# RikVoorhaar/tt-sketch

Hardware: AMD Instinct MI355X
Metric: TT-cores sketched/sec (fp64) + achieved MFMA % for d=6 n=200 r=50 stream_sketch (higher is better)
Workload: dtype f64

## Files before the change

### include/ttsk.h

```cpp
#ifndef TTSK_H
#define TTSK_H

#include <stddef.h>
#include <stdint.h>

#ifdef __cplusplus
extern "C" {
#endif

typedef enum {
    TTSK_OK = 0,
    TTSK_ERR_HIP = -1,
    TTSK_ERR_ARG = -2,
    TTSK_ERR_UNSUPPORTED = -3,
    TTSK_ERR_COMM = -4
} ttsk_status;

#define TTSK_NUM_STREAMS 8

int ttsk_init(int device);
int ttsk_shutdown(void);
const char *ttsk_last_error(void);
int ttsk_device_info(char *name, size_t name_len, int *num_cu, size_t *hbm_bytes);
int ttsk_malloc(void **dev, size_t bytes);
int ttsk_free(void *dev);
int ttsk_memset(void *dev, int value, size_t bytes, int stream);
int ttsk_h2d(void *dev, const void *host, size_t bytes, int stream);
int ttsk_d2h(void *host, const void *dev, size_t bytes, int stream);
int ttsk_d2d(void *dst, const void *src, size_t bytes, int stream);
int ttsk_sync(int stream);
int ttsk_stream_wait(int waiter, int signaller);
int ttsk_timer_start(int stream);
int ttsk_timer_stop(int stream, float *ms);
int ttsk_graph_begin(int stream);
int ttsk_graph_end(int stream, void **graph_exec);
int ttsk_graph_launch(void *graph_exec, int stream);
int ttsk_graph_free(void *graph_exec);

typedef struct {
    int64_t batch, M, N, Ko, Ki;
    int64_t a_b, a_m, a_ko, a_ki;
    int64_t b_b, b_ko, b_ki, b_n;
    int64_t c_b, c_m, c_n;
    double alpha;
    int accumulate;
    int split_k;
} ttsk_gemm_desc;
int ttsk_gemm(const ttsk_gemm_desc *desc, const double *A, const double *B, double *C,
              const double *k_scale ,
              int stream);
int ttsk_copy_strided(double *dst, const double *src, int ndim, const int64_t *shape,
                      const int64_t *dst_strides, const int64_t *src_strides, int stream);
int ttsk_axpby(double *y, const double *x, double a, double b, size_t n, int stream);
int ttsk_sum_slices(double *dst, const double *src, int nb, size_t stride, size_t n, int accumulate, int stream);

int ttsk_tt_sketch(int d, const int64_t *n, const int64_t *s, const int64_t *lt, const int64_t *l_lo,
                   const int64_t *l_hi, const int64_t *rt, const int64_t *r_lo, const int64_t *r_hi,
                   const double *const *X, const double *const *DL, const double *const *DR,
                   double *out, int accumulate, int stream);
int ttsk_tt_sketch_batch(int nb, int d, const int64_t *n, const int64_t *s, const int64_t *lt, const int64_t *l_lo,
                         const int64_t *l_hi, const int64_t *rt, const int64_t *r_lo, const int64_t *r_hi,
                         const double *const *X, const double *const *DL, const double *const *DR,
                         double *out, int64_t out_stride, int accumulate, int stream);
int ttsk_tt_sketch_sum(int nb, int d, const int64_t *n, const int64_t *s, const int64_t *lt, const int64_t *l_lo,
                       const int64_t *l_hi, const int64_t *rt, const int64_t *r_lo, const int64_t *r_hi,
                       const double *const *X, const double *const *DL, const double *const *DR,
                       double *out, int accumulate, int stream);
int ttsk_chain_step(int nb, int n, int K1, int A, int A2, int J, const double *const *W, int64_t w_c,
                    const double *const *X, int64_t x_j, int64_t x_k, int64_t x_c, int64_t x_extent,
                    const double *E, double *const *T, double *const *Out, int stream);
int ttsk_chain_step_wide(int nb, int n, int K1, int A, int A2, int J, const double *const *W, int64_t w_c,
                         const double *const *X, int64_t x_j, int64_t x_k, int64_t x_c, int64_t x_extent,
                         const double *E, double *const *T, double *const *Out, int stream);
int ttsk_chain_step_sum(int nb, int n, int K1, int A, int A2, int J, const double *const *W, int64_t w_c,
                        const double *const *X, int64_t x_j, int64_t x_k, int64_t x_c, int64_t x_extent,
                        const double *E, double *T, int64_t t_b, int64_t t_ld, int64_t t_extent,
                        double *const *Out, int stream);
int ttsk_psi_stream(int nb, int J, int K1, int A, const double *const *S, int64_t s_j, const double *const *W,
                    int64_t w_c, double *const *C, int64_t c_j, int accumulate, int stream);
int ttsk_psi_stream_sum(int nb, int J, int K1, int A, const double *S, int64_t s_j, int64_t s_b, const double *W,
                        int64_t w_c, int64_t w_b, double *C, int64_t c_j, int accumulate, int stream);
int ttsk_drm_pack(const double *core, int A, int n, int A2, int stream);
int ttsk_drm_unpack(const double *core);
int ttsk_dense_left_pass(const double *X, int64_t n0, int64_t n1, int64_t n2, int64_t C, int64_t n4, int l,
                         const double *A0, const double *A1t, const double *A2t, const double *A3, double *Z0, double *Z1,
                         double *Z2, double *E3, int stream);
int64_t ttsk_tt_sketch_size(int d, const int64_t *n, const int64_t *l_lo, const int64_t *l_hi,
                            const int64_t *r_lo, const int64_t *r_hi);
int ttsk_prof_enable(int on);
int ttsk_mfma_f64_peak_probe(double *tflops);
int ttsk_ndtri_rate_probe(double *gsamples);
int ttsk_prof_read(int cls, int64_t *launches, double *total_ms, double *flops);
int ttsk_prof_kernel_name(int cls, char *buf, size_t len);

int ttsk_hash_u64(uint64_t *host_vals, size_t n);
int ttsk_inds_to_rand_double(const uint64_t *host_idx, const uint64_t *shape, int m, size_t N,
                             int rank_min, int rank_max, uint64_t seed, double *host_out);
int ttsk_inds_to_normal(const int64_t *host_idx, const uint64_t *shape, int m, size_t N,
                        int rank_min, int rank_max, uint64_t seed, double *host_out );
int ttsk_inds_to_sparse_sign(const int64_t *host_idx, const uint64_t *shape, int m, size_t N,
                             int true_rank, int rank_min, int rank_max, int nnz_per_row,
                             uint64_t seed, int16_t *host_out );
int ttsk_sparse_normal_dev(const int64_t *dev_idx, int64_t row_stride, const int *row_order,
                           const uint64_t *shape, int m, size_t N, int rank_min, int rank_max,
                           uint64_t seed, double *dev_out, int stream);
int ttsk_sparse_normal_table(const uint64_t *shape, int m, int rank_min, int rank_max, uint64_t seed, double *dev_out,
                             int stream);
int ttsk_sparse_sign_dev(const int64_t *dev_idx, int64_t row_stride, const int *row_order,
                         const uint64_t *shape, int m, size_t N, int true_rank, int rank_min,
                         int rank_max, int nnz_per_row, uint64_t seed, double *dev_out, int stream);
int ttsk_sparse_sign_table(const uint64_t *shape, int m, int true_rank, int rank_min, int rank_max, int nnz_per_row, uint64_t seed,
                           double *dev_out, int stream);
int ttsk_fill_normal(double *dev_out, size_t n, uint64_t seed, double scale, int stream);
int ttsk_fill_normal_many(int count, double *const *dev_outs, const size_t *ns, const uint64_t *seeds,
                          const double *scales, int stream);

int ttsk_sparse_ttdrm_step(const double *dev_vin, int64_t rho, const double *dev_core,
                           int64_t n, int64_t rhop, const int64_t *dev_idx_row, size_t N,
                           double *dev_vout, int stream);
int ttsk_sparse_densedrm_gather(const double *dev_mat, int64_t rank, int64_t cols,
                                const int64_t *dev_idx, int64_t row_stride, const int *row_order,
                                const int64_t *shape, int m, size_t N, double *dev_out, int stream);
int ttsk_sparse_psi(const double *dev_val, const int64_t *dev_idx_row, const int64_t *dev_perm, size_t N,
                    const double *dev_Lv, int64_t l, const double *dev_Rv, int64_t r,
                    int64_t n, double *dev_psi, int stream);

int ttsk_tt_gather(const double *const *dev_cores, const int64_t *ranks , const int64_t *shape, int d,
                   const int64_t *dev_idx, int64_t row_stride, const int *row_order, size_t N,
                   const double *dev_val, double *dev_out, double *dev_stats , int stream);
int ttsk_cp_gather(const double *const *dev_factors, int64_t rank, const int64_t *shape, int d,
                   const int64_t *dev_idx, int64_t row_stride, const int *row_order, size_t N,
                   const double *dev_val, double *dev_out, double *dev_stats, int stream);
int ttsk_tucker_gather(const double *dev_core, const double *const *dev_factors, const int64_t *ranks ,
                       const int64_t *shape, int d, const int64_t *dev_idx, int64_t row_stride, const int *row_order,
                       size_t N, const double *dev_val, double *dev_out, double *dev_stats , int stream);

int ttsk_sparse_key_index(const int64_t *shape, int d, const int64_t *dev_idx, int64_t row_stride, const int *row_order, size_t N,
                          const double *dev_val, int max_split, int64_t *dev_keys_sorted, double *dev_vals_sorted,
                          int64_t *dev_splitters, int stream);
int ttsk_sparse_join(const int64_t *dev_keys_sorted, const double *dev_vals_sorted, const int64_t *dev_splitters, size_t N_table,
                     int max_split, const int64_t *shape, int d, const int64_t *dev_qidx, int64_t q_row_stride,
                     const int *q_row_order, size_t Nq, const double *dev_qval, double *dev_out, double *dev_dot, int stream);
int ttsk_dense_join(const double *dev_x, const int64_t *shape, int d, const int64_t *dev_qidx, int64_t q_row_stride,
                    const int *q_row_order, size_t Nq, const double *dev_qval, double *dev_out, double *dev_dot, int stream);
int ttsk_sparse_join_layout(size_t N_table, size_t Nq, int max_split, int64_t *out);

int ttsk_tt_gram(const double *const *dev_cores_a, const int64_t *ranks_a, int K, const double *const *dev_cores_b,
                 const int64_t *ranks_b, int M, const int64_t *shape, int d, double *dev_out, int stream);

int ttsk_gram_round_bonds(const double *const *dev_gl, const double *const *dev_gr, const int64_t *ranks, const int64_t *caps,
                          int count, double eps, double *const *dev_pt, double *const *dev_q, double *const *dev_sigma,
                          int *dev_rank_out, int stream);

int ttsk_op_apply(int K, const double *const *L, const double *const *M, const double *const *C, const int64_t *dims,
                  const int64_t *strides, int64_t l, double *W, int64_t w_cols, int stream);

int ttsk_hadamard_apply(const double *L, const double *X, const double *Y, const int64_t *dims, const int64_t *strides,
                        double *W, int64_t w_cols, int64_t w_off, int stream);

int ttsk_hadamard_close(const double *Wl, const double *U, const double *V, const int64_t *dims, const int64_t *strides, double *out,
                        int accumulate, double *work, int64_t work_doubles, int stream);
int ttsk_hadamard_close_layout(const int64_t *dims, int64_t *out);

int ttsk_op_close(const double *Wl, const double *N, const double *Y, const int64_t *dims, const int64_t *strides, double *out,
                  int accumulate, double *work, int64_t work_doubles, int stream);
int ttsk_op_close_layout(const int64_t *dims, int64_t *out);

int ttsk_op_close_batch(int npairs, const double *const *Wl, const double *const *N, const double *const *Y, const int64_t *dims,
                        const int64_t *strides, const int64_t *ldw, double *const *out, int accumulate, double *work,
                        int64_t work_doubles, int stream);
int ttsk_op_close_batch_layout(int npairs, const int64_t *dims, int64_t *out);

int ttsk_cp_chain_step(const double *L, int64_t ldl, const double *V, int64_t v_k, int64_t v_j, const double *D, double *out,
                       int64_t ldo, int64_t N, int64_t rho, int64_t n, int64_t rho1, int stream);
int ttsk_cp_psi_omega(const double *L, int64_t ldl, const double *R, int64_t ldr, const double *V, int64_t v_k, int64_t v_j,
                      double *psi, const double *R_om, int64_t ld_om, int64_t r_om, double *omega, int64_t N, int64_t l, int64_t n,
                      int64_t r, int stream);

int ttsk_cp_gram(const double *const *dev_a, const int64_t *lda, int64_t N, const double *const *dev_b, const int64_t *ldb,
                 int64_t M, const int64_t *shape, int d, int sym, double *dev_out , int stream);
int ttsk_sum(const double *dev_x, size_t n, double *dev_out, int stream);

int ttsk_tt_dense_stats(const double *dev_L, int64_t M, const double *dev_R, int64_t N, int64_t rho,
                        const double *dev_x, double *dev_out, double *dev_stats , int stream);
int ttsk_tt_dense_stats_ld(const double *dev_L, int64_t M, const double *dev_R, int64_t N, int64_t rho,
                           const double *dev_x, int64_t ld_x, double *dev_out, int64_t ld_out, double *dev_stats,
                           int accumulate, int stream);
int ttsk_sumsq(const double *dev_x, size_t n, double *dev_out, int stream);

int ttsk_sparse_flat_mult(const uint64_t *shape, int m, uint64_t *mult_out);
int ttsk_sparse_mode_order(const int64_t *dev_idx, int64_t row_stride, size_t N, const int *r_rows, const uint64_t *r_shape, int r_m,
                           int mode_row, int64_t n, int64_t *dev_perm, int stream);
int ttsk_sparse_mode_stream(const int64_t *dev_idx, int64_t row_stride, const int64_t *dev_perm, size_t N, const int *l_rows,
                            const uint64_t *l_shape, int l_m, const int *r_rows, const uint64_t *r_shape, int r_m, int mode_row,
                            const double *dev_val, uint64_t *dev_fl, uint64_t *dev_fr, int32_t *dev_j, double *dev_v, int stream);
int ttsk_sparse_mode_stream_u32(const int64_t *dev_idx, int64_t row_stride, const int64_t *dev_perm, size_t N, const int *l_rows,
                            const uint64_t *l_shape, int l_m, const int *r_rows, const uint64_t *r_shape, int r_m, int mode_row,
                            const double *dev_val, uint32_t *dev_fl, uint32_t *dev_fr, int32_t *dev_j, double *dev_v, int stream);
#define TTSK_SG_CHAIN_MAX 8
typedef struct {
    int steps;
    uint64_t rows;
    const double *core[TTSK_SG_CHAIN_MAX];
    int64_t n[TTSK_SG_CHAIN_MAX];
    int rank[TTSK_SG_CHAIN_MAX + 1];
} ttsk_sg_chain;
typedef struct {
    int kind, w, rank_min, src;
    uint64_t mul, seed;
    const double *table;
    int full, nnz;
    const ttsk_sg_chain *chain;
} ttsk_sg_factor;
int ttsk_sparse_gauss_pass(const uint64_t *dev_fl, const uint64_t *dev_fr, const int32_t *dev_j, const double *dev_val, size_t N,
                           int64_t n, const ttsk_sg_factor *A, const ttsk_sg_factor *B, const ttsk_sg_factor *C, int c_left,
                           double *dev_psi, double *dev_omega, int stream);
int ttsk_sparse_gauss_pass_u32(const uint32_t *dev_fl, const uint32_t *dev_fr, const int32_t *dev_j, const double *dev_val, size_t N,
                           int64_t n, const ttsk_sg_factor *A, const ttsk_sg_factor *B, const ttsk_sg_factor *C, int c_left,
                           double *dev_psi, double *dev_omega, int stream);
int ttsk_sparse_sort_mode(const int64_t *dev_idx_row, size_t N, int64_t n, int64_t *dev_perm, int stream);

int ttsk_pinv(const double *dev_omega, int64_t l, int64_t r, double rcond, double *dev_pinv,
              int *host_rank , int stream);
int ttsk_pinv_begin(const double *dev_omega, int64_t l, int64_t r, double rcond, double *dev_pinv, int stream);
int ttsk_pinv_end(const double *dev_omega, int64_t l, int64_t r, double rcond, double *dev_pinv,
                  int *host_rank , int stream);
int ttsk_svd_small(const double *dev_A, int64_t m, int64_t n, double *dev_US, double *dev_S, double *dev_Vt,
                   int stream);
int ttsk_triu(double *dev_A, int64_t m, int64_t n, int stream);
int ttsk_qr_thin(double *dev_A, int64_t m, int64_t n, int stream);
int ttsk_orth_step(const double *dev_psi, int64_t m, int64_t r2, const double *dev_omega, int64_t l, double *dev_q,
                   int stream);
int ttsk_pinv_batch_deferred(int count, const double *const *dev_omegas, int64_t l, int64_t r, double *const *dev_pinvs,
                             int stream);
int ttsk_orth_step_pinv(const double *dev_psi, int64_t m, int64_t r2, const double *dev_pinv, int64_t l, double *dev_q,
                        int stream);
int ttsk_deferred_status(int stream, int *host_flag);
int ttsk_tt_orth_sketch(int d, const int64_t *n, const int64_t *s, const int64_t *lt, const int64_t *rt,
                        const double *const *X, const double *const *DL, const double *const *DR,
                        double *const *cores_out, double *const *omega_out, int stream);
int ttsk_tt_orth_sketch_batch(int count, int d, const int64_t *n, const int64_t *s, const int64_t *lt, const int64_t *rt,
                              const double *const *X, const double *const *DL, const double *const *DR,
                              double *const *cores_out, double *const *omega_out, int *dev_status, int stream);

int ttsk_dense_first_pass(const double *dev_x, int64_t n0, int64_t Q, int64_t T, const double *dev_c, int64_t ll,
                          const double *dev_p, int64_t r, double *dev_z, double *dev_u, int stream);

int ttsk_pinv_batch(int count, const double *const *dev_omegas, int64_t l, int64_t r, double *const *dev_pinvs, int stream);
int ttsk_tt_assemble(int d, const int64_t *n, const int64_t *lr, const int64_t *rr, const double *const *dev_psi,
                     const double *const *dev_omega, double *const *dev_cores_out, double *const *dev_work, int direction,
                     int stream);
int ttsk_tt_assemble_batch(int count, int d, const int64_t *n, const int64_t *lr, const int64_t *rr,
                           const double *const *dev_psi , const double *const *dev_omega ,
                           double *const *dev_cores_out , double *const *dev_work ,
                           int direction, int stream);
int ttsk_comm_unique_id(void *host_id128);
int ttsk_comm_init(const void *host_id128, int rank, int nranks);
int ttsk_comm_allreduce_sum(double *dev_buf, size_t n, int stream);
int ttsk_comm_reduce_sum(double *dev_buf, size_t n, int root, int stream);
int ttsk_comm_allgather(const double *dev_send, double *dev_recv, size_t n, int stream);
int ttsk_comm_allreduce_max(double *dev_buf, size_t n, int stream);
int ttsk_comm_destroy(void);

#ifdef __cplusplus
}
#endif
#endif
```

### tt_sketch_amd/_native.py

```python
import ctypes
import os
import re
from ctypes import POINTER, Structure, c_char_p, c_double, c_float, c_int, c_int64, c_size_t, c_uint64, c_void_p
from typing import NamedTuple, Optional

_HERE = os.path.dirname(os.path.abspath(__file__))
LIB_PATH = os.environ.get("TTSK_LIB") or os.path.join(_HERE, "libttsk.so")
HEADER_PATH = os.path.join(os.path.dirname(_HERE), "include", "ttsk.h")

TTSK_ERR_ARG = -2
TTSK_ERR_UNSUPPORTED = -3
NUM_STREAMS = 8


class TtskError(RuntimeError):
    """A HIP / RCCL level failure inside libttsk."""


class TtskUnsupported(TtskError):
    """The fused kernel does not cover this shape (caller composes from ttsk_gemm)."""


class GemmDesc(Structure):
    _fields_ = [(n, c_int64) for n in
                ("batch", "M", "N", "Ko", "Ki", "a_b", "a_m", "a_ko", "a_ki",
                 "b_b", "b_ko", "b_ki", "b_n", "c_b", "c_m", "c_n")] + [
        ("alpha", c_double), ("accumulate", c_int), ("split_k", c_int)]


_lib = None


def declared_symbols():
    with open(HEADER_PATH) as f:
        text = f.read()
    return sorted(set(re.findall(r"\b(ttsk_[a-z0-9_]+)\s*\(", text)))


QUEUE = "queue"
FORK_NEXT = "queue, +1"
FORK_ALL = "queue, all"
DRAIN_FIRST = "drain first"
DRAIN_LAST = "drain last"
_QUEUEING = (QUEUE, FORK_NEXT, FORK_ALL)


class Entry(NamedTuple):
    argtypes: list
    role: Optional[str] = None
    restype: type = c_int


P, I, S, I64, U64 = c_void_p, c_int, c_size_t, c_int64, c_uint64
_CHAIN = [I, I, I, I, I, I, POINTER(P), I64, POINTER(P), I64, I64, I64, I64, P]
_MODE_STREAM = [P, I64, P, S, POINTER(I), POINTER(U64), I, POINTER(I), POINTER(U64), I, I, P, P, P, P, P, I]
_GAUSS_PASS = [P, P, P, P, S, I64, P, P, P, I, P, P, I]
ENTRY_POINTS = {
    "ttsk_init": Entry([I]),
    "ttsk_shutdown": Entry([]),
    "ttsk_last_error": Entry([], restype=c_char_p),
    "ttsk_device_info": Entry([c_char_p, S, POINTER(I), POINTER(S)]),
    "ttsk_malloc": Entry([POINTER(P), S]),
    "ttsk_free": Entry([P]),
    "ttsk_memset": Entry([P, I, S, I], QUEUE),
    "ttsk_h2d": Entry([P, P, S, I], DRAIN_LAST),
    "ttsk_d2h": Entry([P, P, S, I], DRAIN_LAST),
    "ttsk_d2d": Entry([P, P, S, I], QUEUE),
    "ttsk_sync": Entry([I], DRAIN_FIRST),
    "ttsk_stream_wait": Entry([I, I]),
    "ttsk_timer_start": Entry([I], QUEUE),
    "ttsk_timer_stop": Entry([I, POINTER(c_float)]),
    "ttsk_graph_begin": Entry([I]),
    "ttsk_graph_end": Entry([I, POINTER(P)]),
    "ttsk_graph_launch": Entry([P, I], QUEUE),
    "ttsk_graph_free": Entry([P]),
    "ttsk_gemm": Entry([POINTER(GemmDesc), P, P, P, P, I], QUEUE),
    "ttsk_copy_strided": Entry([P, P, I, POINTER(I64), POINTER(I64), POINTER(I64), I], QUEUE),
    "ttsk_axpby": Entry([P, P, c_double, c_double, S, I], QUEUE),
    "ttsk_sum_slices": Entry([P, P, I, S, S, I, I], QUEUE),
    "ttsk_tt_sketch": Entry([I] + [POINTER(I64)] * 8 + [POINTER(P)] * 3 + [P, I, I], FORK_NEXT),
    "ttsk_tt_sketch_batch": Entry([I, I] + [POINTER(I64)] * 8 + [POINTER(P)] * 3 + [P, I64, I, I], FORK_NEXT),
    "ttsk_tt_sketch_sum": Entry([I, I] + [POINTER(I64)] * 8 + [POINTER(P)] * 3 + [P, I, I], FORK_NEXT),
    "ttsk_chain_step": Entry(_CHAIN + [POINTER(P), POINTER(P), I], QUEUE),
    "ttsk_chain_step_wide": Entry(_CHAIN + [POINTER(P), POINTER(P), I], QUEUE),
    "ttsk_chain_step_sum": Entry(_CHAIN + [P, I64, I64, I64, POINTER(P), I], QUEUE),
    "ttsk_psi_stream": Entry([I, I, I, I, POINTER(P), I64, POINTER(P), I64, POINTER(P), I64, I, I], QUEUE),
    "ttsk_psi_stream_sum": Entry([I, I, I, I, P, I64, I64, P, I64, I64, P, I64, I, I], QUEUE),
    "ttsk_drm_pack": Entry([P, I, I, I, I], DRAIN_LAST),
    "ttsk_drm_unpack": Entry([P]),
    "ttsk_dense_left_pass": Entry([P, I64, I64, I64, I64, I64, I, P, P, P, P, P, P, P, P, I], QUEUE),
    "ttsk_tt_sketch_size": Entry([I] + [POINTER(I64)] * 5, restype=I64),
    "ttsk_prof_enable": Entry([I]),
    "ttsk_mfma_f64_peak_probe": Entry([POINTER(c_double)]),
    "ttsk_ndtri_rate_probe": Entry([POINTER(c_double)]),
    "ttsk_prof_read": Entry([I, POINTER(I64), POINTER(c_double), POINTER(c_double)]),
    "ttsk_prof_kernel_name": Entry([I, c_char_p, S]),
    "ttsk_hash_u64": Entry([P, S]),
    "ttsk_inds_to_rand_double": Entry([P, P, I, S, I, I, U64, P]),
    "ttsk_inds_to_normal": Entry([P, P, I, S, I, I, U64, P]),
    "ttsk_inds_to_sparse_sign": Entry([P, P, I, S, I, I, I, I, U64, P]),
    "ttsk_sparse_normal_dev": Entry([P, I64, POINTER(I), POINTER(U64), I, S, I, I, U64, P, I], QUEUE),
    "ttsk_sparse_normal_table": Entry([POINTER(U64), I, I, I, U64, P, I], QUEUE),
    "ttsk_sparse_sign_dev": Entry([P, I64, POINTER(I), POINTER(U64), I, S, I, I, I, I, U64, P, I], QUEUE),
    "ttsk_sparse_sign_table": Entry([POINTER(U64), I, I, I, I, I, U64, P, I], QUEUE),
    "ttsk_fill_normal": Entry([P, S, U64, c_double, I], QUEUE),
    "ttsk_fill_normal_many": Entry([I, POINTER(P), POINTER(S), POINTER(U64), POINTER(c_double), I], QUEUE),
    "ttsk_sparse_ttdrm_step": Entry([P, I64, P, I64, I64, P, S, P, I], QUEUE),
    "ttsk_sparse_densedrm_gather": Entry([P, I64, I64, P, I64, POINTER(I), POINTER(I64), I, S, P, I], QUEUE),
    "ttsk_sparse_psi": Entry([P, P, P, S, P, I64, P, I64, I64, P, I], QUEUE),
    "ttsk_tt_gather": Entry([POINTER(P), POINTER(I64), POINTER(I64), I, P, I64, POINTER(I), S, P, P, P, I], QUEUE),
    "ttsk_cp_gather": Entry([POINTER(P), I64, POINTER(I64), I, P, I64, POINTER(I), S, P, P, P, I], QUEUE),
    "ttsk_tucker_gather": Entry([P, POINTER(P), POINTER(I64), POINTER(I64), I, P, I64, POINTER(I), S, P, P, P, I], QUEUE),
    "ttsk_sparse_key_index": Entry([POINTER(I64), I, P, I64, POINTER(I), S, P, I, P, P, P, I], QUEUE),
    "ttsk_sparse_join": Entry([P, P, P, S, I, POINTER(I64), I, P, I64, POINTER(I), S, P, P, P, I], QUEUE),
    "ttsk_dense_join": Entry([P, POINTER(I64), I, P, I64, POINTER(I), S, P, P, P, I], QUEUE),
    "ttsk_sparse_join_layout": Entry([S, S, I, POINTER(I64)]),
    "ttsk_tt_gram": Entry([POINTER(P), POINTER(I64), I, POINTER(P), POINTER(I64), I, POINTER(I64), I, P, I], QUEUE),
    "ttsk_gram_round_bonds": Entry([POINTER(P), POINTER(P), POINTER(I64), POINTER(I64), I, c_double, POINTER(P), POINTER(P), POINTER(P), P, I], QUEUE),
    "ttsk_op_apply": Entry([I, POINTER(P), POINTER(P), POINTER(P), POINTER(I64), POINTER(I64), I64, P, I64, I], QUEUE),
    "ttsk_hadamard_apply": Entry([P, P, P, POINTER(I64), POINTER(I64), P, I64, I64, I], QUEUE),
    "ttsk_hadamard_close": Entry([P, P, P, POINTER(I64), POINTER(I64), P, I, P, I64, I], QUEUE),
    "ttsk_hadamard_close_layout": Entry([POINTER(I64), POINTER(I64)]),
    "ttsk_op_close": Entry([P, P, P, POINTER(I64), POINTER(I64), P, I, P, I64, I], QUEUE),
    "ttsk_op_close_layout": Entry([POINTER(I64), POINTER(I64)]),
    "ttsk_op_close_batch": Entry([I, POINTER(P), POINTER(P), POINTER(P), POINTER(I64), POINTER(I64), POINTER(I64), POINTER(P), I, P, I64, I], QUEUE),
    "ttsk_op_close_batch_layout": Entry([I, POINTER(I64), POINTER(I64)]),
    "ttsk_cp_chain_step": Entry([P, I64, P, I64, I64, P, P, I64, I64, I64, I64, I64, I], QUEUE),
    "ttsk_cp_psi_omega": Entry([P, I64, P, I64, P, I64, I64, P, P, I64, I64, P, I64, I64, I64, I64, I], QUEUE),
    "ttsk_cp_gram": Entry([POINTER(P), POINTER(I64), I64, POINTER(P), POINTER(I64), I64, POINTER(I64), I, I, P, I], QUEUE),
    "ttsk_sum": Entry([P, S, P, I], QUEUE),
    "ttsk_tt_dense_stats": Entry([P, I64, P, I64, I64, P, P, P, I], QUEUE),
    "ttsk_tt_dense_stats_ld": Entry([P, I64, P, I64, I64, P, I64, P, I64, P, I, I], QUEUE),
    "ttsk_sumsq": Entry([P, S, P, I], QUEUE),
    "ttsk_sparse_flat_mult": Entry([POINTER(U64), I, POINTER(U64)]),
    "ttsk_sparse_mode_order": Entry([P, I64, S, POINTER(I), POINTER(U64), I, I, I64, P, I], QUEUE),
    "ttsk_sparse_mode_stream": Entry(_MODE_STREAM, QUEUE),
    "ttsk_sparse_mode_stream_u32": Entry(_MODE_STREAM, QUEUE),
    "ttsk_sparse_gauss_pass": Entry(_GAUSS_PASS, QUEUE),
    "ttsk_sparse_gauss_pass_u32": Entry(_GAUSS_PASS, QUEUE),
    "ttsk_sparse_sort_mode": Entry([P, S, I64, P, I], QUEUE),
    "ttsk_pinv": Entry([P, I64, I64, c_double, P, POINTER(I), I], QUEUE),
    "ttsk_pinv_begin": Entry([P, I64, I64, c_double, P, I], QUEUE),
    "ttsk_pinv_end": Entry([P, I64, I64, c_double, P, POINTER(I), I], QUEUE),
    "ttsk_svd_small": Entry([P, I64, I64, P, P, P, I], QUEUE),
    "ttsk_triu": Entry([P, I64, I64, I], QUEUE),
    "ttsk_qr_thin": Entry([P, I64, I64, I], QUEUE),
    "ttsk_orth_step": Entry([P, I64, I64, P, I64, P, I], QUEUE),
    "ttsk_pinv_batch_deferred": Entry([I, POINTER(P), I64, I64, POINTER(P), I], QUEUE),
    "ttsk_orth_step_pinv": Entry([P, I64, I64, P, I64, P, I], QUEUE),
    "ttsk_deferred_status": Entry([I, POINTER(I)], DRAIN_FIRST),
    "ttsk_tt_orth_sketch": Entry([I] + [POINTER(I64)] * 4 + [POINTER(P)] * 5 + [I], FORK_NEXT),
    "ttsk_tt_orth_sketch_batch": Entry([I, I] + [POINTER(I64)] * 4 + [POINTER(P)] * 5 + [P, I], FORK_ALL),
    "ttsk_dense_first_pass": Entry([P, I64, I64, I64, P, I64, P, I64, P, P, I], QUEUE),
    "ttsk_pinv_batch": Entry([I, POINTER(P), I64, I64, POINTER(P), I], QUEUE),
    "ttsk_tt_assemble": Entry([I] + [POINTER(I64)] * 3 + [POINTER(P)] * 4 + [I, I], FORK_ALL),
    "ttsk_tt_assemble_batch": Entry([I, I] + [POINTER(I64)] * 3 + [POINTER(P)] * 4 + [I, I], QUEUE),
    "ttsk_comm_unique_id": Entry([P]),
    "ttsk_comm_init": Entry([P, I, I]),
    "ttsk_comm_allreduce_sum": Entry([P, S, I], QUEUE),
    "ttsk_comm_reduce_sum": Entry([P, S, I, I], QUEUE),
    "ttsk_comm_allgather": Entry([P, P, S, I], QUEUE),
    "ttsk_comm_allreduce_max": Entry([P, S, I], QUEUE),
    "ttsk_comm_destroy": Entry([]),
}
del P, I, S, I64, U64


def ptr_array(arrays):
    return (c_void_p * len(arrays))(*[a.ptr for a in arrays])


def i64_array(values):
    return (c_int64 * len(values))(*[int(v) for v in values])


def _bind(lib):
    missing = [s for s in declared_symbols() if not hasattr(lib, s)]
    if missing:
        raise TtskError(f"{LIB_PATH} does not export {missing}")
    for name, e in ENTRY_POINTS.items():
        fn = getattr(lib, name)
        fn.argtypes = e.argtypes
        fn.restype = e.restype


def lib():
    global _lib
    if _lib is None:
        if not os.path.exists(LIB_PATH):
            raise TtskError(
                f"{LIB_PATH} not found: build it with `python -c 'import __graft_entry__ as g; g.build()'`; "
                "tt_sketch_amd has no CPU fallback")
        handle = ctypes.CDLL(LIB_PATH, mode=ctypes.RTLD_GLOBAL)
        _bind(handle)
        _lib = handle
    return _lib


def check(rc):
    if rc == 0:
        return
    msg = lib().ttsk_last_error().decode(errors="replace")
    if rc == TTSK_ERR_ARG:
        raise ValueError(msg)
    if rc == TTSK_ERR_UNSUPPORTED:
        raise TtskUnsupported(msg)
    raise TtskError(msg)


_sync_epoch = 0
_stream_gen = [0] * NUM_STREAMS
_dirty = set()


def sync_epoch() -> int:
    return _sync_epoch


def dirty_snapshot() -> dict:
    out = {}
    for s in _dirty:
        t = _joined_into.get(s, s)
        out[t] = _stream_gen[t]
    return out


def drained_since(stream: int, gen: int) -> bool:
    return _stream_gen[stream] > gen


_joined_into = {}


def _mark(name, args):
    e = ENTRY_POINTS.get(name)
    if e is not None and e.role in _QUEUEING:
        s = int(args[-1])
        if 0 <= s < NUM_STREAMS:
            _dirty.add(s)
            _joined_into.pop(s, None)
            helpers = ((s + 1) % NUM_STREAMS,) if e.role == FORK_NEXT else \
                (tuple(h for h in range(NUM_STREAMS) if h != s) if e.role == FORK_ALL else ())
            for h in helpers:
                if h not in _dirty or _joined_into.get(h) == s:
                    _joined_into[h] = s
                _dirty.add(h)


def _drained(s):
    _stream_gen[s] += 1
    _dirty.discard(s)
    _joined_into.pop(s, None)
    for h, into in list(_joined_into.items()):
        if into == s:
            _stream_gen[h] += 1
            _dirty.discard(h)
            del _joined_into[h]


def call(name, *args):
    global _sync_epoch
    _mark(name, args)
    check(getattr(lib(), name)(*args))
    role = ENTRY_POINTS[name].role
    if role in (DRAIN_FIRST, DRAIN_LAST):
        s = int(args[0 if role == DRAIN_FIRST else -1])
        if s < 0:
            _sync_epoch += 1
            for i in range(NUM_STREAMS):
                _stream_gen[i] += 1
            _dirty.clear()
            _joined_into.clear()
        elif s < NUM_STREAMS:
            _drained(s)
```

### tt_sketch_amd/csrc/chain_fused.h

```cpp
#pragma once
#include "chain_stages.h"

namespace ttsk {

#ifdef TTSK_LAB
#define CF_DIAG(bit) (a.diag & (bit))
#define CF_STAMP(i) do { if (a.stamps && blockIdx.x == 0 && lane == 0 && k - k_beg < 8) a.stamps[((k - k_beg) * CD_WAVES + w) * 8 + (i)] = __builtin_amdgcn_s_memtime(); } while (0)
#else
#define CF_DIAG(bit) 0
#define CF_STAMP(i) do { } while (0)
#endif
#define CF_BARRIER() do { if (!CF_DIAG(4)) lds_barrier(); } while (0)

template <int NQF, int STRQ, int NNF, int STRN, int D, bool WT, int EBUF, int UNR, int KIND, int APC = 0>
__device__ __forceinline__ void cf_piece(const ChainStep &a, const double *Wl, const double *El, int tile, int q0, int prob,
                                         int g, int k_beg, int k_end, int KB1, int w, int lane)
{
    const int x16 = lane & 15, kq = lane >> 4;
    const int AP = APC ? APC : a.AP, A2P = a.A2P;
    const int j0 = 16 * tile;
    const bool jok = j0 + x16 < a.J;
    const uint32_t xlane = !CF_DIAG(1) ? (uint32_t)(((int64_t)(j0 + x16) * a.x_j + (int64_t)kq * a.x_c) * 8) : OOB_OFF;
    const __amdgpu_buffer_rsrc_t rx = make_rsrc(uniform_ptr(a.X[prob]), a.x_extent * 8);
    const uint32_t xstep = __builtin_amdgcn_readfirstlane((uint32_t)(4 * a.x_c * 8));
    const uint32_t kstep = __builtin_amdgcn_readfirstlane((uint32_t)(a.x_k * 8));
    static_assert(UNR % D == 0, "the unrolled body must keep the ring slots static");
    const int ITER = KB1 / UNR;
    auto xload = [&](uint32_t so) -> double { return ld8(rx, xlane, __builtin_amdgcn_readfirstlane(so)); };
    double ring[D];
#pragma unroll
    for (int d = 0; d < D; ++d) ring[d] = xload((uint32_t)k_beg * kstep + (uint32_t)d * xstep);

    v4d acc2[NNF ? NNF : 1];
    double acc2s[STRN ? STRN : 1];
#pragma unroll
    for (int p = 0; p < NNF; ++p)
#pragma unroll
        for (int t = 0; t < 4; ++t) acc2[p][t] = 0.0;
#pragma unroll
    for (int q = 0; q < STRN; ++q) acc2s[q] = 0.0;

    const int wl_lane = (kq >> 1) * 2 * AP + 2 * (16 * q0 + x16) + (kq & 1);
    const int ws_lane = (kq >> 1) * 2 * AP + 2 * (16 * (q0 + NQF) + (x16 & 3)) + (kq & 1);
    const int el_lane = e_frag_lane(x16, kq, A2P);
    const int es_col = 16 * NNF + (x16 & 3);
    const int es_lane = e_strip_lane(kq, A2P);

    __amdgpu_buffer_rsrc_t rt;
    if constexpr (WT) rt = make_rsrc(uniform_ptr(a.T[prob]), a.t_extent * 8);

    for (int k = k_beg; k < k_end; ++k) {
        v4d acc1[NQF ? NQF : 1];
        double acc1s[STRQ ? STRQ : 1];
#pragma unroll
        for (int p = 0; p < NQF; ++p)
#pragma unroll
            for (int t = 0; t < 4; ++t) acc1[p][t] = 0.0;
#pragma unroll
        for (int q = 0; q < STRQ; ++q) acc1s[q] = 0.0;

        CF_STAMP(0);
        double af[NQF ? NQF : 1], sf[STRQ ? STRQ : 1];
        auto wfetch = [&](const double *wrun, int u, double (&f)[NQF ? NQF : 1], double (&g)[STRQ ? STRQ : 1]) {
#pragma unroll
            for (int p = 0; p < NQF; ++p) f[p] = LDS_UNPAIRED(wrun[wl_lane + u * 4 * AP + 32 * p]);
#pragma unroll
            for (int q = 0; q < STRQ; ++q) g[q] = wrun[ws_lane + u * 4 * AP + 8 * q];
        };
        wfetch(Wl, 0, af, sf);
        uint32_t so = (uint32_t)k * kstep + (uint32_t)D * xstep;
        auto kblock = [&](const double *wrun, int u, bool wrap) {
            const int d = u % D;
            double afn[NQF ? NQF : 1], sfn[STRQ ? STRQ : 1];
            wfetch(wrun, u + 1, afn, sfn);
            const double bf = ring[d];
#pragma unroll
            for (int p = 0; p < NQF; ++p) acc1[p] = mfma16(af[p], bf, acc1[p]);
#pragma unroll
            for (int q = 0; q < STRQ; ++q) acc1s[q] = mfma4(sf[q], bf, acc1s[q]);
            if (wrap) so = (uint32_t)(k + 1) * kstep;
            ring[d] = xload(so);
            so += xstep;
#pragma unroll
            for (int p = 0; p < NQF; ++p) af[p] = afn[p];
#pragma unroll
            for (int q = 0; q < STRQ; ++q) sf[q] = sfn[q];
        };
        for (int it = 0; it < ITER; ++it) {
            const double *wrun = Wl + it * UNR * 4 * AP;
            const bool last = it == ITER - 1;
#pragma unroll
            for (int u = 0; u < UNR; ++u) kblock(wrun, u, last && u + D == UNR);
        }
        if constexpr (WT) {
            const int64_t nJ = (int64_t)a.n * a.J;
            const int a0 = 16 * q0;
            const uint32_t tl = jok ? (uint32_t)(((int64_t)(a0 + kq) * nJ + (int64_t)k * a.J + j0 + x16) * 8) : OOB_OFF;
#pragma unroll
            for (int p = 0; p < NQF; ++p)
#pragma unroll
                for (int t = 0; t < 4; ++t)
                    st8(rt, (jok && a0 + 16 * p + 4 * t + kq < a.A) ? tl + (uint32_t)((16 * p + 4 * t) * nJ * 8) : OOB_OFF, acc1[p][t]);
#pragma unroll
            for (int q = 0; q < STRQ; ++q)
                st8(rt, (jok && a0 + 16 * NQF + 4 * q + kq < a.A) ? tl + (uint32_t)((16 * NQF + 4 * q) * nJ * 8) : OOB_OFF, acc1s[q]);
        }
        CF_STAMP(1);
        CF_BARRIER();
        CF_STAMP(2);

        {
            const double *eb = El + (EBUF == 2 ? (k & 1) * a.eunits * 2 : 0) + q0 * 16 * A2P;
            double bf[NNF ? NNF : 1], bs[STRN ? STRN : 1];
            int el0 = el_lane, es0 = es_lane + e_image_at(0, es_col, A2P);
            asm volatile("" : "+v"(el0), "+v"(es0));
            auto efetch = [&](int kap, double (&f)[NNF ? NNF : 1], double (&g)[STRN ? STRN : 1]) {
#pragma unroll
                for (int nn = 0; nn < NNF; ++nn) f[nn] = LDS_UNPAIRED(eb[el0 + kap * 4 * A2P + 32 * nn]);
#pragma unroll
                for (int q = 0; q < STRN; ++q) g[q] = eb[es0 + kap * 4 * A2P + 8 * q];
            };
            double bf2[NNF ? NNF : 1], bs2[STRN ? STRN : 1];
            efetch(0, bf, bs);
            constexpr int KB2C = 4 * NQF + STRQ;
#pragma unroll
            for (int kap = 0; kap < KB2C; ++kap) {
                const int p = kap >> 2, t = kap & 3;
                const double af2 = p < NQF ? acc1[p < NQF ? p : 0][t] : acc1s[t < STRQ ? t : 0];
                if (kap & 1) {
                    if (kap + 1 < KB2C) efetch(kap + 1, bf, bs);
                    __builtin_amdgcn_sched_barrier(0);
#pragma unroll
                    for (int nn = 0; nn < NNF; ++nn) acc2[nn] = mfma16(af2, bf2[nn], acc2[nn]);
#pragma unroll
                    for (int q = 0; q < STRN; ++q) acc2s[q] = mfma4(af2, bs2[q], acc2s[q]);
                } else {
                    if (kap + 1 < KB2C) efetch(kap + 1, bf2, bs2);
                    __builtin_amdgcn_sched_barrier(0);
#pragma unroll
                    for (int nn = 0; nn < NNF; ++nn) acc2[nn] = mfma16(af2, bf[nn], acc2[nn]);
#pragma unroll
                    for (int q = 0; q < STRN; ++q) acc2s[q] = mfma4(af2, bs[q], acc2s[q]);
                }
            }
        }
        CF_STAMP(3);
        CF_BARRIER();
        CF_STAMP(4);
    }

    double *slab = a.slab + ((int64_t)prob * a.wpp + g) * a.J * a.A2;
    if constexpr (KIND == CD_FIRST) __syncthreads();
    int ln = lane;
    if constexpr (APC != 0) asm volatile("v_mbcnt_lo_u32_b32 %0, -1, 0\n\tv_mbcnt_hi_u32_b32 %0, -1, %0" : "=v"(ln));
    const int sx = ln & 15, sk = ln >> 4;
#pragma unroll
    for (int nn = 0; nn < NNF; ++nn)
#pragma unroll
        for (int t = 0; t < 4; ++t) {
            const int j = j0 + 4 * t + sk, col = 16 * nn + sx;
            if (j < a.J && col < a.A2) {
                double *p = slab + (int64_t)j * a.A2 + col;
                *p = KIND == CD_FIRST ? acc2[nn][t] + *p : acc2[nn][t];
            }
        }
#pragma unroll
    for (int q = 0; q < STRN; ++q) {
        const int j = j0 + 4 * ((ln >> 2) & 3) + sk, col = 16 * NNF + 4 * q + (ln & 3);
        if (j < a.J && col < a.A2) {
            double *p = slab + (int64_t)j * a.A2 + col;
            *p = KIND == CD_FIRST ? acc2s[q] + *p : acc2s[q];
        }
    }
    if constexpr (KIND == CD_REST) {
        __threadfence_block();
        __syncthreads();
    }
}

template <int NQF, int STRQ, int NNF, int STRN, int D, bool WT, int EBUF, int UNR, int APC>
__device__ __forceinline__ void cf_rows4(const ChainStep &a, const double *Wl, const double *El, int tile, int prob, int g,
                                         int k_beg, int k_end, int KB1, int w, int lane)
{
    constexpr int NC = 4 * NNF + STRN;
    __builtin_amdgcn_s_setprio(2);
    const int x16 = lane & 15, kq = lane >> 4, n4 = x16 & 3, beta = x16 >> 2;
    constexpr int AP = APC;
    const int A2P = a.A2P;
    const int j0 = 16 * tile;
    const bool jok = j0 + n4 < a.J;
    const uint32_t xlane = !CF_DIAG(1) ? (uint32_t)(((int64_t)(j0 + n4) * a.x_j + (int64_t)kq * a.x_c) * 8) : OOB_OFF;
    const __amdgpu_buffer_rsrc_t rx = make_rsrc(uniform_ptr(a.X[prob]), a.x_extent * 8);
    const uint32_t xstep = __builtin_amdgcn_readfirstlane((uint32_t)(4 * a.x_c * 8));
    const uint32_t kstep = __builtin_amdgcn_readfirstlane((uint32_t)(a.x_k * 8));
    const int ITER = KB1 / UNR;
    auto xload = [&](uint32_t so) -> double { return ld8(rx, xlane, __builtin_amdgcn_readfirstlane(so)); };
    double ring[D];
#pragma unroll
    for (int d = 0; d < D; ++d) ring[d] = xload((uint32_t)k_beg * kstep + (uint32_t)d * xstep);

    double acc2[NC];
#pragma unroll
    for (int c = 0; c < NC; ++c) acc2[c] = 0.0;

    const int wl_lane = (kq >> 1) * 2 * AP + 2 * x16 + (kq & 1);
    const int ws_lane = (kq >> 1) * 2 * AP + 2 * (16 * NQF + n4) + (kq & 1);
    const int el_lane = e_image_at(4 * beta + kq, n4, A2P);
    const int es_lane = e_image_at(kq, n4, A2P);

    __amdgpu_buffer_rsrc_t rt;
    if constexpr (WT) rt = make_rsrc(uniform_ptr(a.T[prob]), a.t_extent * 8);

    for (int k = k_beg; k < k_end; ++k) {
        double acc1[NQF], acc1s[STRQ ? STRQ : 1];
#pragma unroll
        for (int p = 0; p < NQF; ++p) acc1[p] = 0.0;
#pragma unroll
        for (int q = 0; q < STRQ; ++q) acc1s[q] = 0.0;
        CF_STAMP(0);
        uint32_t so = (uint32_t)k * kstep + (uint32_t)D * xstep;
        for (int it = 0; it < ITER; ++it) {
            const double *wrun = Wl + it * UNR * 4 * AP;
            const bool last = it == ITER - 1;
#pragma unroll
            for (int u = 0; u < UNR; ++u) {
                const int d = u % D;
                const double bf = ring[d];
#pragma unroll
                for (int p = 0; p < NQF; ++p) acc1[p] = mfma4(LDS_UNPAIRED(wrun[wl_lane + u * 4 * AP + 32 * p]), bf, acc1[p]);
#pragma unroll
                for (int q = 0; q < STRQ; ++q) acc1s[q] = mfma4(wrun[ws_lane + u * 4 * AP + 8 * q], bf, acc1s[q]);
                if (last && u + D == UNR) so = (uint32_t)(k + 1) * kstep;
                ring[d] = xload(so);
                so += xstep;
            }
        }
        if constexpr (WT) {
            const int64_t nJ = (int64_t)a.n * a.J;
            const uint32_t tl = (uint32_t)(((int64_t)kq * nJ + (int64_t)k * a.J + j0 + n4) * 8);
#pragma unroll
            for (int p = 0; p < NQF; ++p)
                st8(rt, (jok && 16 * p + 4 * beta + kq < a.A) ? tl + (uint32_t)((16 * p + 4 * beta) * nJ * 8) : OOB_OFF, acc1[p]);
#pragma unroll
            for (int q = 0; q < STRQ; ++q)
                st8(rt, (jok && beta == 0 && 16 * NQF + 4 * q + kq < a.A) ? tl + (uint32_t)((16 * NQF + 4 * q) * nJ * 8) : OOB_OFF,
                    acc1s[q]);
        }
        CF_STAMP(1);
        CF_BARRIER();
        CF_STAMP(2);
        {
            const double *eb = El + (EBUF == 2 ? (k & 1) * a.eunits * 2 : 0);
            int el0 = el_lane, es0 = es_lane;
            asm volatile("" : "+v"(el0), "+v"(es0));
#pragma unroll
            for (int p = 0; p < NQF; ++p)
#pragma unroll
                for (int c = 0; c < NC; ++c) acc2[c] = mfma4(acc1[p], eb[el0 + p * 16 * A2P + 8 * c], acc2[c]);
#pragma unroll
            for (int q = 0; q < STRQ; ++q)
#pragma unroll
                for (int c = 0; c < NC; ++c) {
                    const double e = eb[es0 + (8 * NQF + 2 * q) * 2 * A2P + 8 * c];
                    acc2[c] = mfma4(acc1s[q], beta == 0 ? e : 0.0, acc2[c]);
                }
        }
        CF_STAMP(3);
        CF_BARRIER();
        CF_STAMP(4);
    }

    double *slab = a.slab + ((int64_t)prob * a.wpp + g) * a.J * a.A2;
#pragma unroll
    for (int c = 0; c < NC; ++c) {
        double v = acc2[c];
        v += __shfl_xor(v, 4);
        v += __shfl_xor(v, 8);
        const int j = j0 + kq, col = 4 * c + n4;
        if (beta == 0 && j < a.J && col < a.A2) slab[(int64_t)j * a.A2 + col] = v;
    }
}

template <int NQF, int STRQ, int NNF, int STRN, int D, bool WT, int OCC, int EBUF, int UNR = 5 * D, int NWV = 8>
__global__ __launch_bounds__(64 * NWV, NWV == 8 ? 2 * OCC : 1) void chain_step_kernel(ChainStep a)
{
    extern __shared__ double cf_lds[];
    double *Wl = cf_lds;
    double *El = cf_lds + a.ebase;
    const int tid = threadIdx.x, lane = tid & 63, w = tid >> 6;
    constexpr int NT = 64 * NWV;
    int prob, g;
    chain_block_unit(a.xcd_map, a.wpp, prob, g);
    const int k_beg = (int)((int64_t)g * a.n / a.wpp), k_end = (int)((int64_t)(g + 1) * a.n / a.wpp);
    const int KB1 = ((a.K1 + 3) / 4 + UNR - 1) / UNR * UNR;
    const int AP = a.AP, A2P = a.A2P;

    {
        const double *Wp = uniform_ptr(a.W[prob]);
        const __amdgpu_buffer_rsrc_t rw = make_rsrc(Wp, ((int64_t)(a.K1 - 1) * a.w_c + a.A) * 8);
        const int total = 4 * KB1 * AP;
        constexpr int BATCH = 10;
        for (int e0 = tid; e0 < total; e0 += NT * BATCH) {
            double v[BATCH];
#pragma unroll
            for (int u = 0; u < BATCH; ++u) {
                const int e = e0 + NT * u;
                const int c = e / AP, col = e - c * AP;
                v[u] = ld8(rw, (e < total && c < a.K1 && col < a.A) ? (uint32_t)(((int64_t)c * a.w_c + col) * 8) : OOB_OFF, 0);
            }
#pragma unroll
            for (int u = 0; u < BATCH; ++u) {
                const int e = e0 + NT * u;
                const int c = e / AP, col = e - c * AP;
                if (e < total) Wl[(c >> 1) * 2 * AP + 2 * col + (c & 1)] = v[u];
            }
        }
    }

    unsigned pc = 0;
    int li = 0, nl = 1;
    if constexpr (NWV != 8) {
        pc = a.piece[__builtin_amdgcn_readfirstlane(w)];
        li = __builtin_amdgcn_readfirstlane((pc >> 8) & 255);
        nl = a.nload;
    }
    if (NWV == 8 ? w == 7 : __builtin_amdgcn_readfirstlane(pc >> 16) == CD_NONE) {
        if constexpr (NWV != 8) __builtin_amdgcn_s_setprio(3);
#ifdef TTSK_LAB
        if (CF_DIAG(8)) {
            if (li > 0) { __syncthreads(); return; }
            nl = 1;
        }
#endif
        const int NI = CF_DIAG(2) ? 0 : a.eunits >> 6;
        const uint32_t inv = e_image_inv(A2P);
        const int64_t rowstride = (int64_t)a.n * a.A2;
        const int ebuf = a.eunits * 2;
        auto fill_gather = [&](int k) {
            chain_e_fill_gather<false>(a, El + (EBUF == 2 ? (k & 1) * ebuf : 0), k, 0, A2P, inv, rowstride, NI, li, nl, lane);
        };
        const uint32_t lane16 = 16u * (uint32_t)lane;
        auto fill_packed = [&](int k) {
            const char *src = (const char *)(a.Epk + ((int64_t)k * a.eunits + 64 * li) * 2);
            double *dst = El + (EBUF == 2 ? (k & 1) * ebuf : 0);
#pragma unroll 2
            for (int m = li; m < NI; m += nl, src += 1024 * nl)
                __builtin_amdgcn_global_load_lds((const __attribute__((address_space(1))) void *)(src + lane16),
                                                 (__attribute__((address_space(3))) void *)(dst + m * 128), 16, 0, 0);
        };
        const bool packed = a.Epk != nullptr;
        auto fill = [&](int k) {
            if (packed) fill_packed(k);
            else fill_gather(k);
        };
        __syncthreads();
        if constexpr (EBUF == 2) {
            if (k_beg < k_end) fill(k_beg);
            for (int k = k_beg; k < k_end; ++k) {
                asm volatile("s_waitcnt vmcnt(0)" ::: "memory");
                CF_STAMP(1);
                CF_BARRIER();
                CF_STAMP(2);
                if (k + 1 < k_end) fill(k + 1);
                CF_STAMP(3);
                CF_BARRIER();
                CF_STAMP(4);
            }
        } else {
            for (int k = k_beg; k < k_end; ++k) {
                CF_STAMP(0);
                fill(k);
                asm volatile("s_waitcnt vmcnt(0)" ::: "memory");
                CF_STAMP(1);
                CF_BARRIER();
                CF_STAMP(2);
                CF_STAMP(3);
                CF_BARRIER();
                CF_STAMP(4);
            }
        }
        return;
    }
    __syncthreads();
    if constexpr (NWV == 8) {
        if (w >= (a.J + 15) >> 4) return;
        cf_piece<NQF, STRQ, NNF, STRN, D, WT, EBUF, UNR, CD_WHOLE>(a, Wl, El, w, 0, prob, g, k_beg, k_end, KB1, w, lane);
    } else {
        const int kind = __builtin_amdgcn_readfirstlane(pc >> 16), tile = __builtin_amdgcn_readfirstlane(pc & 255);
        constexpr int H = cd_cut(NQF), APC = 16 * NQF + 4 * STRQ;
        if (kind == CD_WHOLE)
            cf_piece<NQF, STRQ, NNF, STRN, D, WT, EBUF, UNR, CD_WHOLE, APC>(a, Wl, El, tile, 0, prob, g, k_beg, k_end, KB1, w, lane);
        else if (kind == CD_FIRST)
            cf_piece<H, 0, NNF, STRN, D, WT, EBUF, UNR, CD_FIRST, APC>(a, Wl, El, tile, 0, prob, g, k_beg, k_end, KB1, w, lane);
        else if (kind == CD_REST)
            cf_piece<NQF - H, STRQ, NNF, STRN, D, WT, EBUF, UNR, CD_REST, APC>(a, Wl, El, tile, H, prob, g, k_beg, k_end, KB1, w, lane);
        else if (kind == CD_ROWS4)
            cf_rows4<NQF, STRQ, NNF, STRN, D, WT, EBUF, UNR, APC>(a, Wl, El, tile, prob, g, k_beg, k_end, KB1, w, lane);
    }
}

inline double *chain_slab_request(int stream, const ChainLaunch &l) { return (double *)scratch(stream, SCRATCH_GEMM, (size_t)l.slab * 8 + 64); }

inline int chain_slab_reduce(hipStream_t st, const double *slab, const ChainLaunch &l, const ChainStepArgs &c)
{
    RReduceArgs r{l.red_chunks, l.red_m, l.red_n, 1, c.nb, (int64_t)c.J, (int64_t)c.A2, 1, 1.0, 0, {}};
    for (int b = 0; b < c.nb; ++b) r.out.C[b] = c.Out[b];
    return launch_r_reduce(st, slab, r);
}

int chain_fused_try(const ChainStepArgs &c, int stream, hipStream_t st, bool force = false);

const double *drm_packed_lookup(const double *E, int A, int n, int A2, int A2P, int eunits);

}
```

### tt_sketch_amd/csrc/chain_fused.hip

```cpp
#include <cstdlib>
#include "chain_fused.h"
#include "prof.h"

namespace ttsk {

int launch_chain_step_a(const ChainStep &a, int nf, int str, bool wt, int ebuf, int unr, int waves, size_t lds, int grid, hipStream_t st);
int launch_chain_step_b(const ChainStep &a, int nf, int str, bool wt, int ebuf, int unr, int waves, size_t lds, int grid, hipStream_t st);
int launch_chain_step_c(const ChainStep &a, int nf, int str, bool wt, int ebuf, int unr, int waves, size_t lds, int grid, hipStream_t st);
int launch_chain_step_d(const ChainStep &a, int nf, int str, bool wt, int ebuf, int unr, int waves, size_t lds, int grid, hipStream_t st);
int launch_chain_step_e(const ChainStep &a, int nf, int str, bool wt, int ebuf, int unr, int waves, size_t lds, int grid, hipStream_t st);

static int launch_chain_step(const ChainStep &a, int nf, int str, bool wt, int ebuf, int unr, int waves, size_t lds, int grid, hipStream_t st)
{
    if (nf <= 2) return launch_chain_step_a(a, nf, str, wt, ebuf, unr, waves, lds, grid, st);
    if (nf <= 4) return launch_chain_step_b(a, nf, str, wt, ebuf, unr, waves, lds, grid, st);
    if (nf == 5) return launch_chain_step_c(a, nf, str, wt, ebuf, unr, waves, lds, grid, st);
    if (nf == 6) return launch_chain_step_d(a, nf, str, wt, ebuf, unr, waves, lds, grid, st);
    return launch_chain_step_e(a, nf, str, wt, ebuf, unr, waves, lds, grid, st);
}

int chain_fused_try(const ChainStepArgs &c, int stream, hipStream_t st, bool force)
{
    const int n_cu = device_num_cu();
    if (n_cu < 1) return TTSK_ERR_HIP;
    ChainFusedPlan p;
    if (!chain_fused_plan(c, n_cu, force, p)) return 0;
    ChainStep &a = p.a;
    a.slab = chain_slab_request(stream, p.l);
    if (!a.slab) return TTSK_ERR_HIP;
    a.Epk = drm_packed_lookup(c.E, c.A, c.n, c.A2, a.A2P, a.eunits);
    ProfBracket prof(st, PROF_CURRENT, p.l.flops,
                     "chain_step_kernel<%d, %d, %d, %d, 5, %s, 1, %d, %d>", p.nq, p.sq, p.nq, p.sq, p.wt ? "true" : "false", p.ebuf, p.unr);
#ifdef TTSK_LAB
    { static int dg = [] { const char *e = getenv("TTSK_CF_DIAG"); return e ? atoi(e) : 0; }(); a.diag = dg; }
    static int stamps_on = [] { const char *e = getenv("TTSK_CF_STAMPS"); return e ? atoi(e) : 0; }();
#else
    constexpr int stamps_on = 0;
#endif
    long long *stamps_dev = nullptr;
    if (stamps_on) {
        if (hipMalloc(&stamps_dev, 8 * CD_WAVES * 8 * 8) != hipSuccess) return TTSK_ERR_HIP;
        (void)hipMemset(stamps_dev, 0, 8 * CD_WAVES * 8 * 8);
        a.stamps = stamps_dev;
    }
    int rc = launch_chain_step(a, p.nq, p.sq, p.wt, p.ebuf, p.unr, p.waves, p.l.lds, p.l.grid, st);
    if (stamps_on) {
        long long h[8 * CD_WAVES * 8];
        (void)hipStreamSynchronize(st);
        (void)hipMemcpy(h, stamps_dev, sizeof(h), hipMemcpyDeviceToHost);
        (void)hipFree(stamps_dev);
        long long t0 = 0;
        for (int i = 0; i < 8 * CD_WAVES * 8; ++i) if (h[i] && (!t0 || h[i] < t0)) t0 = h[i];
        fprintf(stderr, "[cf stamps] workgroup 0: cycles since its first stamp; per slice, wave: start | endA | afterB1 | endB | afterB2\n");
        for (int sl = 0; sl < 8; ++sl)
            for (int w = 0; w < CD_WAVES; ++w) {
                const long long *r = h + (sl * CD_WAVES + w) * 8;
                if (!r[1] && !r[4]) continue;
                fprintf(stderr, "  slice %d wave %d: %8lld %8lld %8lld %8lld %8lld\n", sl, w, r[0] ? r[0] - t0 : -1, r[1] - t0, r[2] - t0,
                        r[3] - t0, r[4] - t0);
            }
    }
    if (rc == TTSK_OK) rc = chain_slab_reduce(st, a.slab, p.l, c);
    return rc == TTSK_OK ? 1 : (rc == 1 ? 0 : rc);
}

}

using namespace ttsk;

extern "C" int ttsk_chain_step(int nb, int n, int K1, int A, int A2, int J, const double *const *W, int64_t w_c,
                               const double *const *X, int64_t x_j, int64_t x_k, int64_t x_c, int64_t x_extent,
                               const double *E, double *const *T, double *const *Out, int stream)
{
    TTSK_STREAM(st, stream);
    TTSK_ARG(W && X && E && Out && nb >= 1, "ttsk_chain_step: NULL argument");
    ChainStepArgs c{nb, n, K1, A, A2, J, W, w_c, X, x_j, x_k, x_c, x_extent, E, T, Out};
    const int rc = chain_fused_try(c, stream, st, true);
    if (rc == 0) {
        set_error("ttsk_chain_step: shape (n=%d K1=%d A=%d A2=%d J=%d nb=%d) is not covered by the fused kernel", n, K1, A,
                  A2, J, nb);
        return TTSK_ERR_UNSUPPORTED;
    }
    return rc < 0 ? rc : TTSK_OK;
}
```

### tt_sketch_amd/csrc/chain_sum.h

```cpp
#pragma once
#include <cstddef>
#include "chain_fused.h"

namespace ttsk {

#ifdef TTSK_LAB
#define CS_DIAG(bit) (a.diag & (bit))
#else
#define CS_DIAG(bit) 0
#endif

template <int JS, int KB1, int NA>
struct CsPre {
    static constexpr int JP = 4 * JS, KP = 4 * KB1;
    static constexpr int GMAX = (KP * JP + 127) / 128;
    double Wf[NA][KB1];
    uint32_t goff[GMAX];
    int glds[GMAX];
    int esrc[CS_DMAMAX];
    int tw[NA], twt[NA];
    uint32_t tg[NA], tgt[NA];
    __amdgpu_buffer_rsrc_t rx, rt;
    uint32_t kstep, tkstep, tastep;
    int gl_lane, gl_tile, tl_lane, el_lane, es_lane;
    int k_beg, k_end, tb;
    double greg0[GMAX];
};

template <int JS, int KB1, int NA, bool WT>
__device__ __forceinline__ void cs_prologue(const ChainSumS &a, const ChainSumRole ro, const double *Wterm, const double *Xterm,
                                            double *lds, const int g, const int rr, const int w, const int lane, CsPre<JS, KB1, NA> &P)
{
    constexpr int JP = 4 * JS, KP = 4 * KB1, GMAX = CsPre<JS, KB1, NA>::GMAX;
    const int x16 = lane & 15, kq = lane >> 4;
    const int RP = a.RP, A2P = a.A2P, KB2 = a.KB2;
#ifdef TTSK_LAB
#define CS_PSTAMP(i) do { if (a.stamps && blockIdx.x == 0 && lane == 0) a.stamps[((4 * 8) + w) * 8 + (i)] = __builtin_amdgcn_s_memtime(); } while (0)
#else
#define CS_PSTAMP(i) do { } while (0)
#endif
    P.k_beg = rr * a.kbase + (rr < a.krem ? rr : a.krem);
    P.k_end = P.k_beg + a.kbase + (rr < a.krem ? 1 : 0);
    const int tb = g * a.tpw + ro.term;
    const bool tv = tb < a.nb;
    P.tb = tb;
    const int wpt = a.wpt;
    const int lt = wpt == 8 ? 0 : (wpt == 4 ? w >> 2 : w >> 1), part = w - lt * wpt;
    const int gt = g * a.tpw + lt;
    const int per = a.per;
    const int gu = a.gu;
#pragma unroll
    for (int u = 0; u < GMAX; ++u) {
        const uint32_t e = (uint32_t)(part * per + u * 64 + lane);
        const bool in = u < gu && u * 64 + lane < per && e < (uint32_t)(KP * JP);
        uint32_t c, j;
        if constexpr (KP == JP) {
            const uint32_t q = e / (uint32_t)JP, r = e - q * (uint32_t)JP;
            c = a.c_fast ? r : q;
            j = a.c_fast ? q : r;
        } else {
            c = a.c_fast ? e % (uint32_t)KP : e / (uint32_t)JP;
            j = a.c_fast ? e / (uint32_t)KP : e % (uint32_t)JP;
        }
        uint32_t off = j * a.x_j8 + c * a.x_c8;
        asm volatile("" : "+v"(off));
        P.goff[u] = (in && gt < a.nb && c < (uint32_t)a.K1 && j < (uint32_t)a.J) ? off : OOB_OFF;
        P.glds[u] = in ? lt * (KP * JP) + (int)(c * JP + j) : -1;
    }
    P.rx = make_rsrc(uniform_ptr(Xterm), a.x_extent * 8);
    P.kstep = (uint32_t)(a.x_k * 8);
    double greg[GMAX];
#pragma unroll
    for (int u = 0; u < GMAX; ++u) greg[u] = ld8(P.rx, P.goff[u], __builtin_amdgcn_readfirstlane((uint32_t)P.k_beg * P.kstep));
    asm volatile("" ::: "memory");
    CS_PSTAMP(0);
    {
        const double *Wp = uniform_ptr(Wterm);
        const __amdgpu_buffer_rsrc_t rw = make_rsrc(Wp, ((int64_t)(a.K1 - 1) * a.w_c + a.A) * 8);
        uint32_t wrow = (uint32_t)kq * a.w_c8;
        const uint32_t wstep = 4u * a.w_c8;
        uint32_t rmask[KB1];
#pragma unroll
        for (int kb = 0; kb < KB1; ++kb) rmask[kb] = 4 * kb + kq < a.K1 ? 0u : OOB_OFF;
#pragma unroll
        for (int p = 0; p < NA; ++p) {
            const int col = 16 * (ro.at0 + p) + x16;
            uint32_t w0 = (wrow + 8u * (uint32_t)col) | ((tv && p < ro.na && col < a.A) ? 0u : OOB_OFF);
            asm volatile("" : "+v"(w0));
#pragma unroll
            for (int kb = 0; kb < KB1; ++kb) P.Wf[p][kb] = ld8(rw, w0 | rmask[kb], (uint32_t)kb * wstep);
        }
    }
    CS_PSTAMP(1);
    {
        const int rowstride = a.n * a.A2;
#pragma unroll
        for (int i = 0; i < CS_DMAMAX; ++i) {
            const EUnit un = e_image_unit(64u * (uint32_t)(w + 8 * i) + (uint32_t)lane, a.e_inv, a.A, a.A2, A2P);
            P.esrc[i] = (un.row * rowstride + un.col) * 8;
        }
    }
    CS_PSTAMP(2);
    P.gl_lane = ro.term * (KP * JP) + kq * JP + (x16 & 3);
    P.gl_tile = ro.term * (KP * JP) + kq * JP + x16;
    P.tl_lane = (kq >> 1) * 2 * RP + 2 * x16 + (kq & 1);
    P.el_lane = e_frag_lane(x16, kq, A2P);
    P.es_lane = e_strip_lane(kq, A2P) + e_image_at(0, 16 * a.NNF + (x16 & 3), A2P);
    const int beta = (lane >> 2) & 3, j4 = lane & 3;
    if constexpr (WT) P.rt = make_rsrc(a.T, a.t_extent * 8);
#pragma unroll
    for (int p = 0; p < NA; ++p) {
        const int ai = 16 * (ro.at0 + p) + 4 * beta + kq;
        P.tw[p] = (p < ro.na && ai < 4 * KB2) ? (ai >> 1) * 2 * RP + 2 * (ro.term * JP + j4) + (ai & 1) : -1;
        if constexpr (WT) {
            uint32_t o = (uint32_t)tb * a.t_b8 + (uint32_t)ai * a.t_a8 + 8u * (uint32_t)j4;
            asm volatile("" : "+v"(o));
            P.tg[p] = (tv && p < ro.na && ai < a.A) ? o : OOB_OFF;
        } else P.tg[p] = OOB_OFF;
        const int at = 16 * (ro.at0 + p) + kq;
        P.twt[p] = p < ro.na ? (at >> 1) * 2 * RP + 2 * (ro.term * JP + x16) + (at & 1) : -1;
        if constexpr (WT) {
            uint32_t o = (uint32_t)tb * a.t_b8 + (uint32_t)at * a.t_a8 + 8u * (uint32_t)x16;
            asm volatile("" : "+v"(o));
            P.tgt[p] = (tv && p < ro.na) ? o : OOB_OFF;
        } else P.tgt[p] = OOB_OFF;
    }
    P.tkstep = (uint32_t)(a.t_ld * 8);
    P.tastep = 4u * a.t_a8;
    CS_PSTAMP(3);
#pragma unroll
    for (int u = 0; u < GMAX; ++u) P.greg0[u] = greg[u];
#undef CS_PSTAMP
}

template <int JS, int KB1, int NA, bool WT, int RT, int CT, int SR, int NS>
__device__ __forceinline__ void cs_wave(const ChainSumS &a, const ChainSumRole ro, const CsPre<JS, KB1, NA> &P, double *lds,
                                        const int g, const int rr, const int w, const int lane)
{
    constexpr int JP = 4 * JS, KP = 4 * KB1;
    constexpr int GMAX = CsPre<JS, KB1, NA>::GMAX;
    constexpr int NST = WT ? NA * (4 * (JS / 4) + JS % 4) : 0;
    constexpr bool HS = SR > 0;
#ifdef TTSK_LAB
    if (a.stamps && blockIdx.x == 0 && lane == 0) a.stamps[((5 * 8) + w) * 8 + 0] = __builtin_amdgcn_s_memtime();
#endif
    double *TL = lds, *EL = lds + a.ebase, *GL = lds + a.gbase;
    const int x16 = lane & 15, kq = lane >> 4;
    const int k_beg = P.k_beg, k_end = P.k_end;
    const int RP = a.RP, A2P = a.A2P, KB2 = a.KB2;
    const int NI = a.eunits >> 6;
    const int beta = (lane >> 2) & 3, j4 = lane & 3;
    const int tb = P.tb;
    const auto &Wf = P.Wf;
    const auto &tw = P.tw; const auto &twt = P.twt; const auto &tg = P.tg; const auto &tgt = P.tgt;
    const __amdgpu_buffer_rsrc_t rt = P.rt;
    const uint32_t tkstep = P.tkstep, tastep = P.tastep;
    const int gl_lane = P.gl_lane, gl_tile = P.gl_tile, tl_lane = P.tl_lane, el_lane = P.el_lane, es_lane = P.es_lane;
    double greg[GMAX];
    auto g_load = [&](int k) {
#pragma unroll
        for (int u = 0; u < GMAX; ++u)
            greg[u] = ld8(P.rx, P.goff[u], __builtin_amdgcn_readfirstlane((uint32_t)k * P.kstep));
    };
    auto g_store = [&]() {
#pragma unroll
        for (int u = 0; u < GMAX; ++u)
            if (P.glds[u] >= 0) GL[P.glds[u]] = greg[u];
    };
    auto e_fill = [&](int k) {
        const char *Ek = (const char *)uniform_ptr(a.E + (int64_t)k * a.A2);
#pragma unroll
        for (int i = 0; i < CS_DMAMAX; ++i)
            if (w + 8 * i < NI)
                __builtin_amdgcn_global_load_lds((const __attribute__((address_space(1))) void *)(Ek + (uint32_t)P.esrc[i]),
                                                 (__attribute__((address_space(3))) void *)(EL + (w + 8 * i) * 128), 16, 0, 0);
    };

    v4d acc2[RT ? RT : 1][CT ? CT : 1];
    double acc2s[HS ? SR : 1][HS ? NS : 1];
#pragma unroll
    for (int r = 0; r < RT; ++r)
#pragma unroll
        for (int c = 0; c < CT; ++c)
#pragma unroll
            for (int t = 0; t < 4; ++t) acc2[r][c][t] = 0.0;
    if constexpr (HS) {
#pragma unroll
        for (int r = 0; r < SR; ++r)
#pragma unroll
            for (int s = 0; s < NS; ++s) acc2s[r][s] = 0.0;
    }

    {
#ifdef TTSK_LAB
        if (a.stamps && blockIdx.x == 0 && lane == 0) a.stamps[((4 * 8) + w) * 8 + 4] = __builtin_amdgcn_s_memtime();
#endif
#pragma unroll
        for (int u = 0; u < GMAX; ++u)
            if (P.glds[u] >= 0) GL[P.glds[u]] = P.greg0[u];
#ifdef TTSK_LAB
        if (a.stamps && blockIdx.x == 0 && lane == 0) a.stamps[((4 * 8) + w) * 8 + 5] = __builtin_amdgcn_s_memtime();
#endif
        __syncthreads();
#ifdef TTSK_LAB
        if (a.stamps && blockIdx.x == 0 && lane == 0) a.stamps[((4 * 8) + w) * 8 + 7] = __builtin_amdgcn_s_memtime();
#endif
    }

#ifdef TTSK_LAB
#define CS_STAMP(i) do { if (a.stamps && blockIdx.x == 0 && lane == 0 && k - k_beg < 8) a.stamps[((k - k_beg) * 8 + w) * 8 + (i)] = __builtin_amdgcn_s_memtime(); } while (0)
#else
#define CS_STAMP(i) do { } while (0)
#endif
    for (int k = k_beg; k < k_end; ++k) {
        CS_STAMP(0);
        if (!(CS_DIAG(1))) e_fill(k);
        if (k + 1 < k_end && !(CS_DIAG(8))) g_load(k + 1);
        if (!(CS_DIAG(2))) {
            constexpr int NT = JS / 4, NR = JS % 4;
            v4d acc1[NA][NT ? NT : 1];
            double acc1s[NA][NR ? NR : 1];
#pragma unroll
            for (int p = 0; p < NA; ++p) {
#pragma unroll
                for (int q = 0; q < NT; ++q)
#pragma unroll
                    for (int t = 0; t < 4; ++t) acc1[p][q][t] = 0.0;
#pragma unroll
                for (int q = 0; q < NR; ++q) acc1s[p][q] = 0.0;
            }
            double gt[2][NT ? NT : 1], gs[2][NR ? NR : 1];
            auto gfetch = [&](int kb, int set) {
#pragma unroll
                for (int q = 0; q < NT; ++q) gt[set][q] = GL[gl_tile + 4 * kb * JP + 16 * q];
#pragma unroll
                for (int q = 0; q < NR; ++q) gs[set][q] = GL[gl_lane + 4 * kb * JP + 16 * NT + 4 * q];
            };
            gfetch(0, 0);
#pragma unroll
            for (int kb = 0; kb < KB1; ++kb) {
                const int set = kb & 1;
                if constexpr (NT > 0) acc1[0][0] = mfma16(Wf[0][kb], gt[set][0], acc1[0][0]);
                else acc1s[0][0] = mfma4(Wf[0][kb], gs[set][0], acc1s[0][0]);
                __builtin_amdgcn_sched_barrier(0);
                if (kb + 1 < KB1) gfetch(kb + 1, set ^ 1);
                __builtin_amdgcn_sched_barrier(0);
#pragma unroll
                for (int p = 0; p < NA; ++p) {
#pragma unroll
                    for (int q = 0; q < NT; ++q)
                        if (p + q > 0) acc1[p][q] = mfma16(Wf[p][kb], gt[set][q], acc1[p][q]);
#pragma unroll
                    for (int q = 0; q < NR; ++q)
                        if (NT > 0 || p + q > 0) acc1s[p][q] = mfma4(Wf[p][kb], gs[set][q], acc1s[p][q]);
                }
            }
            uint32_t so = 0;
            if constexpr (WT) so = __builtin_amdgcn_readfirstlane((uint32_t)k * tkstep);
#pragma unroll
            for (int p = 0; p < NA; ++p) {
                if (p < ro.na) {
#pragma unroll
                    for (int q = 0; q < NT; ++q)
#pragma unroll
                        for (int t = 0; t < 4; ++t)
                            if (twt[p] >= 0 && 16 * (ro.at0 + p) + 4 * t + kq < 4 * KB2) TL[twt[p] + t * 4 * RP + 32 * q] = acc1[p][q][t];
                    if (tw[p] >= 0) {
#pragma unroll
                        for (int q = 0; q < NR; ++q) TL[tw[p] + 2 * (16 * NT + 4 * q)] = acc1s[p][q];
                    }
                }
                if constexpr (WT) {
#pragma unroll
                    for (int q = 0; q < NT; ++q)
#pragma unroll
                        for (int t = 0; t < 4; ++t)
                            st8s(rt, (tgt[p] != OOB_OFF && 16 * (ro.at0 + p) + 4 * t + kq < a.A && 16 * q + x16 < a.J)
                                         ? tgt[p] + (uint32_t)t * tastep + 128u * q : OOB_OFF, so, acc1[p][q][t]);
#pragma unroll
                    for (int q = 0; q < NR; ++q)
                        st8s(rt, (tg[p] != OOB_OFF && 16 * NT + 4 * q + j4 < a.J) ? tg[p] + 8u * (16 * NT + 4 * q) : OOB_OFF, so, acc1s[p][q]);
                }
            }
        } else if constexpr (WT) {
#pragma unroll
            for (int s = 0; s < NST; ++s) st8(rt, OOB_OFF, 0.0);
        }
        CS_STAMP(1);
        if (k + 1 < k_end) {
            if constexpr (WT) asm volatile("s_waitcnt vmcnt(%0)" :: "n"(NST + GMAX) : "memory");
            else asm volatile("s_waitcnt vmcnt(%0)" :: "n"(GMAX) : "memory");
        } else {
            if constexpr (WT) asm volatile("s_waitcnt vmcnt(%0)" :: "n"(NST) : "memory");
            else asm volatile("s_waitcnt vmcnt(0)" ::: "memory");
        }
        CS_STAMP(2);
        if (!(CS_DIAG(16))) lds_barrier();
        CS_STAMP(3);
        if (k + 1 < k_end) {
            if constexpr (WT) asm volatile("s_waitcnt vmcnt(%0)" :: "n"(NST) : "memory");
            else asm volatile("s_waitcnt vmcnt(0)" ::: "memory");
            g_store();
        }

        constexpr bool SMALL = RT * CT <= 3;
        if constexpr (SMALL) { if (!(CS_DIAG(64))) __builtin_amdgcn_s_setprio(2); }
        if constexpr (RT * CT > 0) {
            double af[2][RT], bf[2][CT];
            int tl0 = tl_lane + 32 * ro.rt0, el0 = el_lane + 32 * ro.ct0;
            asm volatile("" : "+v"(tl0), "+v"(el0));
            const double *tp = TL + tl0, *ep = EL + el0;
            const int tstep = 4 * RP, estep = 4 * A2P;
            auto fetch = [&](int set) {
#pragma unroll
                for (int r = 0; r < RT; ++r) af[set][r] = LDS_UNPAIRED(tp[32 * r]);
#pragma unroll
                for (int c = 0; c < CT; ++c) bf[set][c] = LDS_UNPAIRED(ep[32 * c]);
                tp += tstep;
                ep += estep;
            };
            auto step = [&](int set, bool more) {
                acc2[0][0] = mfma16(af[set][0], bf[set][0], acc2[0][0]);
                __builtin_amdgcn_sched_barrier(0);
                if (more) fetch(set ^ 1);
                __builtin_amdgcn_sched_barrier(0);
#pragma unroll
                for (int r = 0; r < RT; ++r)
#pragma unroll
                    for (int c = 0; c < CT; ++c)
                        if (r + c > 0) acc2[r][c] = mfma16(af[set][r], bf[set][c], acc2[r][c]);
            };
            if (!(CS_DIAG(4))) {
                fetch(0);
                const int pairs = (KB2 - 1) >> 1;
                for (int i = 0; i < pairs; ++i) {
                    step(0, true);
                    step(1, true);
                }
                if (KB2 & 1) step(0, false);
                else { step(0, true); step(1, false); }
            }
        }
        if constexpr (HS) {
            double as[2][SR], bs[2][NS];
            int ts0 = tl_lane, es0 = es_lane;
            asm volatile("" : "+v"(ts0), "+v"(es0));
            const double *tp = TL + ts0, *ep = EL + es0;
            const int tstep = 4 * RP, estep = 4 * A2P;
            auto fetch = [&](int set) {
#pragma unroll
                for (int r = 0; r < SR; ++r) as[set][r] = LDS_UNPAIRED(tp[32 * r]);
#pragma unroll
                for (int s = 0; s < NS; ++s) bs[set][s] = ep[8 * s];
                tp += tstep;
                ep += estep;
            };
            auto step = [&](int set, bool more) {
                acc2s[0][0] = mfma4(as[set][0], bs[set][0], acc2s[0][0]);
                __builtin_amdgcn_sched_barrier(0);
                if (more) fetch(set ^ 1);
                __builtin_amdgcn_sched_barrier(0);
#pragma unroll
                for (int r = 0; r < SR; ++r)
#pragma unroll
                    for (int s = 0; s < NS; ++s)
                        if (r + s > 0) acc2s[r][s] = mfma4(as[set][r], bs[set][s], acc2s[r][s]);
            };
            if (!(CS_DIAG(4))) {
                fetch(0);
                const int pairs = (KB2 - 1) >> 1;
                for (int i = 0; i < pairs; ++i) {
                    step(0, true);
                    step(1, true);
                }
                if (KB2 & 1) step(0, false);
                else { step(0, true); step(1, false); }
            }
        }
        if constexpr (SMALL) __builtin_amdgcn_s_setprio(0);
        CS_STAMP(4);
        if (!(CS_DIAG(16))) lds_barrier();
        CS_STAMP(5);
    }
#undef CS_STAMP

    const __amdgpu_buffer_rsrc_t rs = make_rsrc(a.slab, (int64_t)a.nb * a.slab_t8);
    const uint32_t slab0 = (uint32_t)rr * a.slab_r8;
    auto rowoff = [&](int row) -> uint32_t {
        const int lt2 = row / JP, j = row - lt2 * JP, t2 = g * a.tpw + lt2;
        return (lt2 < a.tpw && t2 < a.nb && j < a.J) ? slab0 + (uint32_t)t2 * a.slab_t8 + (uint32_t)(j * a.A2) * 8u : OOB_OFF;
    };
#pragma unroll
    for (int r = 0; r < RT; ++r)
#pragma unroll
        for (int t = 0; t < 4; ++t) {
            const uint32_t ro8 = rowoff(16 * (ro.rt0 + r) + 4 * t + kq);
#pragma unroll
            for (int c = 0; c < CT; ++c) {
                const int col = 16 * (ro.ct0 + c) + x16;
                st8(rs, (ro8 != OOB_OFF && col < a.A2) ? ro8 + 8u * (uint32_t)col : OOB_OFF, acc2[r][c][t]);
            }
        }
    if constexpr (HS) {
#pragma unroll
        for (int r = 0; r < SR; ++r) {
            const uint32_t ro8 = rowoff(16 * r + 4 * beta + kq);
#pragma unroll
            for (int s = 0; s < NS; ++s) {
                const int col = 16 * a.NNF + 4 * s + j4;
                st8(rs, (ro8 != OOB_OFF && col < a.A2) ? ro8 + 8u * (uint32_t)col : OOB_OFF, acc2s[r][s]);
            }
        }
    }
}

template <int JS, int KB1, int NA, bool WT>
__global__ __launch_bounds__(512, 2) void chain_sum_kernel(ChainSum a)
{
    extern __shared__ double cs_lds[];
    const int lane = threadIdx.x & 63;
    const int w = __builtin_amdgcn_readfirstlane((int)(threadIdx.x >> 6));
#ifdef TTSK_LAB
    if (a.s.stamps && blockIdx.x == 0 && lane == 0) a.s.stamps[w * 8 + 6] = __builtin_amdgcn_s_memtime();
#endif
    int g, rr;
    if (a.s.xcd_map) {
        const int x = blockIdx.x & 7, idx = blockIdx.x >> 3;
        const int q = (int)(((uint32_t)idx * (uint32_t)a.s.inv_ng) >> 20);
        g = idx - q * a.s.ngroups;
        rr = x + 8 * q;
    } else {
        rr = (int)(((uint32_t)blockIdx.x * (uint32_t)a.s.inv_ng) >> 20);
        g = (int)blockIdx.x - rr * a.s.ngroups;
    }
    typedef const __attribute__((address_space(4))) char *karg_t;
    typedef const __attribute__((address_space(4))) unsigned long long *karg64_t;
    const karg_t kp = (karg_t)__builtin_amdgcn_kernarg_segment_ptr();
    const unsigned long long rbits = *(karg64_t)(kp + offsetof(ChainSum, role) + 8 * w);
    ChainSumRole ro;
    ro.term = (unsigned char)(rbits & 0xff); ro.at0 = (unsigned char)((rbits >> 8) & 0xff); ro.na = (unsigned char)((rbits >> 16) & 0xff);
    ro.body = (unsigned char)((rbits >> 24) & 0xff); ro.rt0 = (unsigned char)((rbits >> 32) & 0xff); ro.ct0 = (unsigned char)((rbits >> 40) & 0xff);
    ro.pad0 = ro.pad1 = 0;
    const int wpt = a.s.wpt;
    const int tb = g * a.s.tpw + ro.term, gt = g * a.s.tpw + (wpt == 8 ? 0 : (wpt == 4 ? w >> 2 : w >> 1));
    const double *Wterm = (const double *)*(karg64_t)(kp + offsetof(ChainSum, W) + 8 * (tb < a.s.nb ? tb : 0));
    const double *Xterm = (const double *)*(karg64_t)(kp + offsetof(ChainSum, X) + 8 * (gt < a.s.nb ? gt : 0));
#ifdef TTSK_LAB
    if (a.s.stamps && blockIdx.x == 0 && lane == 0) a.s.stamps[(4 * 8 + w) * 8 + 6] = __builtin_amdgcn_s_memtime();
#endif
    CsPre<JS, KB1, NA> pre;
    cs_prologue<JS, KB1, NA, WT>(a.s, ro, Wterm, Xterm, cs_lds, g, rr, w, lane, pre);
#define CS_CALL(RT_, CT_, SR_, NS_) cs_wave<JS, KB1, NA, WT, RT_, CT_, SR_, NS_>(a.s, ro, pre, cs_lds, g, rr, w, lane)
#define CS_RECT(RT_, CT_) case 16 * RT_ + CT_: CS_CALL(RT_, CT_, 0, 0); break;
#define CS_STRIP(SR_, NS_) case 128 + 16 * SR_ + NS_: CS_CALL(0, 0, SR_, NS_); break;
    switch (ro.body) {
    CS_RECT_BODIES(CS_RECT)
    CS_STRIP_BODIES(CS_STRIP)
    default: CS_CALL(0, 0, 0, 0); break;
    }
#undef CS_CALL
#undef CS_RECT
#undef CS_STRIP
#ifdef TTSK_LAB
    if (a.s.stamps && blockIdx.x == 0 && lane == 0) a.s.stamps[w * 8 + 7] = __builtin_amdgcn_s_memtime();
#endif
}

int chain_sum_try(const ChainSumArgs &c, int stream, hipStream_t st, bool force = false);
int launch_chain_sum_2(const ChainSum &a, bool wt, size_t lds, int grid, hipStream_t st);
int launch_chain_sum_4(const ChainSum &a, bool wt, size_t lds, int grid, hipStream_t st);

}
```

### tt_sketch_amd/csrc/chain_sum.hip

```cpp
#include <cstdlib>
#include "chain_sum.h"
#include "prof.h"

namespace ttsk {

int chain_sum_try(const ChainSumArgs &cc, int stream, hipStream_t st, bool force)
{
    const ChainStepArgs &c = cc.s;
    const int n_cu = device_num_cu();
    if (n_cu < 1) return TTSK_ERR_HIP;
    ChainSumPlan p;
    if (!chain_sum_plan(cc, n_cu, force, p)) return 0;
    ChainSum &ka = p.ka;
    ChainSumS &a = ka.s;
    a.slab = chain_slab_request(stream, p.l);
    if (!a.slab) return TTSK_ERR_HIP;
    ProfBracket prof(st, PROF_CURRENT, p.l.flops,
                     "chain_sum_kernel<5, 5, NA, %s>", p.wt ? "true" : "false");
#ifdef TTSK_LAB
    { static int dg = [] { const char *e = getenv("TTSK_CS_DIAG"); return e ? atoi(e) : 0; }(); a.diag = dg; }
    static int stamps_on = [] { const char *e = getenv("TTSK_CS_STAMPS"); return e ? atoi(e) : 0; }();
    long long *stamps_dev = nullptr;
    if (stamps_on) {
        if (hipMalloc(&stamps_dev, 8 * 8 * 8 * 8) != hipSuccess) return TTSK_ERR_HIP;
        (void)hipMemset(stamps_dev, 0, 8 * 8 * 8 * 8);
        a.stamps = stamps_dev;
    }
#endif
    int rc = p.na_run <= 2 ? launch_chain_sum_2(ka, p.wt, p.l.lds, p.l.grid, st) : launch_chain_sum_4(ka, p.wt, p.l.lds, p.l.grid, st);
    if (rc != TTSK_OK) set_error("chain_sum_kernel launch failed");
#ifdef TTSK_LAB
    if (stamps_on) {
        long long h[8 * 8 * 8];
        (void)hipStreamSynchronize(st);
        (void)hipMemcpy(h, stamps_dev, sizeof(h), hipMemcpyDeviceToHost);
        (void)hipFree(stamps_dev);
        long long t0 = 0;
        for (int i = 0; i < 8 * 8 * 8; ++i) if (h[i] && (!t0 || h[i] < t0)) t0 = h[i];
        for (int w = 0; w < 8; ++w)
            fprintf(stderr, "[cs stamps] wave %d: kernel entry -> first slice %lld cycles, last barrier -> behind the stores %lld cycles\n", w,
                    h[w * 8 + 0] - h[w * 8 + 6], h[w * 8 + 7] - h[(3 * 8 + w) * 8 + 5]);
        for (int w = 0; w < 8; ++w) {
            const long long *r = h + (4 * 8 + w) * 8, e = h[w * 8 + 6];
            fprintf(stderr, "[cs stamps] prologue wave %d: picked %lld | G issued %lld | W issued %lld | E offsets %lld | lane offsets %lld | body entered %lld | G store begins %lld | G stored %lld | barrier passed %lld | first slice %lld\n", w,
                    r[6] - e, r[0] - e, r[1] - e, r[2] - e, r[3] - e, h[(5 * 8 + w) * 8] - e, r[4] - e, r[5] - e, r[7] - e, h[w * 8 + 0] - e);
        }
        fprintf(stderr, "[cs stamps] workgroup 0, cycles since its first stamp; slice, wave (body): start | endA | dma landed | afterB1 | endB | afterB2\n");
        for (int sl = 0; sl < 4; ++sl)
            for (int w = 0; w < 8; ++w) {
                const long long *r = h + (sl * 8 + w) * 8;
                fprintf(stderr, "  slice %d wave %d (%02x): %8lld %8lld %8lld %8lld %8lld %8lld\n", sl, w, ka.role[w].body, r[0] - t0, r[1] - t0, r[2] - t0,
                        r[3] - t0, r[4] - t0, r[5] - t0);
            }
    }
#endif
    if (rc == TTSK_OK) rc = chain_slab_reduce(st, a.slab, p.l, c);
    return rc == TTSK_OK ? 1 : rc;
}

}

using namespace ttsk;

extern "C" int ttsk_chain_step_sum(int nb, int n, int K1, int A, int A2, int J, const double *const *W, int64_t w_c,
                                   const double *const *X, int64_t x_j, int64_t x_k, int64_t x_c, int64_t x_extent,
                                   const double *E, double *T, int64_t t_b, int64_t t_ld, int64_t t_extent,
                                   double *const *Out, int stream)
{
    TTSK_STREAM(st, stream);
    TTSK_ARG(W && X && E && Out && nb >= 1, "ttsk_chain_step_sum: NULL argument");
    ChainSumArgs c{{nb, n, K1, A, A2, J, W, w_c, X, x_j, x_k, x_c, x_extent, E, nullptr, Out}, T, t_b, t_ld, t_extent};
    const int rc = chain_sum_try(c, stream, st, true);
    if (rc == 0) {
        set_error("ttsk_chain_step_sum: shape (n=%d K1=%d A=%d A2=%d J=%d nb=%d) is not covered by the stacked-terms kernel", n,
                  K1, A, A2, J, nb);
        return TTSK_ERR_UNSUPPORTED;
    }
    return rc < 0 ? rc : TTSK_OK;
}
```

### tt_sketch_amd/csrc/chain_wide.h

```cpp
#pragma once
#include "chain_fused.h"

namespace ttsk {

template <int NQF, int STRQ, int NNF, int STRN, bool WT, int UNR, int MT>
__device__ __forceinline__ void cw_compute(const ChainWide &a, const double *Wl, const double *El, const int prob, const int unit,
                                           const int a0, const int cnt, const int k_beg, const int k_end, const int t0, const int t1)
{
    constexpr int D = 5;
    constexpr int AP = 16 * NQF + 4 * STRQ;
    static_assert(UNR % D == 0, "the unrolled body must keep the ring slots static");
    const int lane = threadIdx.x & 63, x16 = lane & 15, kq = lane >> 4;
    const int KB1 = ((a.K1 + 3) / 4 + UNR - 1) / UNR * UNR;
    const int A2P = a.A2P;
    int j0[MT];
    bool jok[MT];
    uint32_t xlane[MT];
    j0[0] = 16 * t0;
    if constexpr (MT == 2) j0[1] = 16 * t1;
#pragma unroll
    for (int m = 0; m < MT; ++m) {
        jok[m] = j0[m] + x16 < a.J;
        xlane[m] = (uint32_t)(((int64_t)(j0[m] + x16) * a.x_j + (int64_t)kq * a.x_c) * 8);
    }
    const __amdgpu_buffer_rsrc_t rx = make_rsrc(uniform_ptr(a.X[prob]), a.x_extent * 8);
    const uint32_t xstep = __builtin_amdgcn_readfirstlane((uint32_t)(4 * a.x_c * 8));
    const uint32_t kstep = __builtin_amdgcn_readfirstlane((uint32_t)(a.x_k * 8));
    const int ITER = KB1 / UNR;
    double ring[MT][D];
#pragma unroll
    for (int d = 0; d < D; ++d)
#pragma unroll
        for (int m = 0; m < MT; ++m)
            ring[m][d] = ld8(rx, xlane[m], __builtin_amdgcn_readfirstlane((uint32_t)k_beg * kstep + (uint32_t)d * xstep));

    v4d acc2[MT][NNF ? NNF : 1];
    double acc2s[MT][STRN ? STRN : 1];
#pragma unroll
    for (int m = 0; m < MT; ++m) {
#pragma unroll
        for (int p = 0; p < NNF; ++p)
#pragma unroll
            for (int t = 0; t < 4; ++t) acc2[m][p][t] = 0.0;
#pragma unroll
        for (int q = 0; q < STRN; ++q) acc2s[m][q] = 0.0;
    }

    const int wl_lane = (kq >> 1) * 2 * AP + 2 * x16 + (kq & 1);
    const int ws_lane = (kq >> 1) * 2 * AP + 2 * (16 * NQF + (x16 & 3)) + (kq & 1);
    const int el_lane = e_frag_lane(x16, kq, A2P);
    const int es_col = 16 * NNF + (x16 & 3);
    const int es_lane = e_strip_lane(kq, A2P);

    __amdgpu_buffer_rsrc_t rt;
    if constexpr (WT) rt = make_rsrc(uniform_ptr(a.T[prob]), a.t_extent * 8);

    for (int k = k_beg; k < k_end; ++k) {
        v4d acc1[MT][NQF ? NQF : 1];
        double acc1s[MT][STRQ ? STRQ : 1];
#pragma unroll
        for (int m = 0; m < MT; ++m) {
#pragma unroll
            for (int p = 0; p < NQF; ++p)
#pragma unroll
                for (int t = 0; t < 4; ++t) acc1[m][p][t] = 0.0;
#pragma unroll
            for (int q = 0; q < STRQ; ++q) acc1s[m][q] = 0.0;
        }
        double af[NQF ? NQF : 1], sf[STRQ ? STRQ : 1];
        auto wfetch = [&](const double *wrun, int u, double (&f)[NQF ? NQF : 1], double (&g)[STRQ ? STRQ : 1]) {
#pragma unroll
            for (int p = 0; p < NQF; ++p) f[p] = LDS_UNPAIRED(wrun[wl_lane + u * 4 * AP + 32 * p]);
#pragma unroll
            for (int q = 0; q < STRQ; ++q) g[q] = wrun[ws_lane + u * 4 * AP + 8 * q];
        };
        wfetch(Wl, 0, af, sf);
        uint32_t so = (uint32_t)k * kstep + (uint32_t)D * xstep;
        auto kblock = [&](const double *wrun, int u, bool wrap) {
            const int d = u % D;
            double afn[NQF ? NQF : 1], sfn[STRQ ? STRQ : 1];
            wfetch(wrun, u + 1, afn, sfn);
            double bf[MT];
#pragma unroll
            for (int m = 0; m < MT; ++m) bf[m] = ring[m][d];
#pragma unroll
            for (int p = 0; p < NQF; ++p)
#pragma unroll
                for (int m = 0; m < MT; ++m) acc1[m][p] = mfma16(af[p], bf[m], acc1[m][p]);
#pragma unroll
            for (int q = 0; q < STRQ; ++q)
#pragma unroll
                for (int m = 0; m < MT; ++m) acc1s[m][q] = mfma4(sf[q], bf[m], acc1s[m][q]);
            if (wrap) so = (uint32_t)(k + 1) * kstep;
            const uint32_t sou = __builtin_amdgcn_readfirstlane(so);
#pragma unroll
            for (int m = 0; m < MT; ++m) ring[m][d] = ld8(rx, xlane[m], sou);
            so += xstep;
#pragma unroll
            for (int p = 0; p < NQF; ++p) af[p] = afn[p];
#pragma unroll
            for (int q = 0; q < STRQ; ++q) sf[q] = sfn[q];
        };
        for (int it = 0; it < ITER; ++it) {
            const double *wrun = Wl + it * UNR * 4 * AP;
            const bool last = it == ITER - 1;
#pragma unroll
            for (int u = 0; u < UNR; ++u) kblock(wrun, u, last && u + D == UNR);
        }
        if constexpr (WT) {
            const int64_t nJ = (int64_t)a.n * a.J;
#pragma unroll
            for (int m = 0; m < MT; ++m) {
                const uint32_t tl = jok[m] ? (uint32_t)((((int64_t)a0 + kq) * nJ + (int64_t)k * a.J + j0[m] + x16) * 8) : OOB_OFF;
#pragma unroll
                for (int p = 0; p < NQF; ++p)
#pragma unroll
                    for (int t = 0; t < 4; ++t)
                        st8(rt, (jok[m] && 16 * p + 4 * t + kq < cnt) ? tl + (uint32_t)((16 * p + 4 * t) * nJ * 8) : OOB_OFF, acc1[m][p][t]);
#pragma unroll
                for (int q = 0; q < STRQ; ++q)
                    st8(rt, (jok[m] && 16 * NQF + 4 * q + kq < cnt) ? tl + (uint32_t)((16 * NQF + 4 * q) * nJ * 8) : OOB_OFF, acc1s[m][q]);
            }
        }
        lds_barrier();
        {
            const double *eb = El + ((a.ebuf2 && (k & 1)) ? a.eunits * 2 : 0);
            double bf[NNF ? NNF : 1], bs[STRN ? STRN : 1];
            int el0 = el_lane, es0 = es_lane + 4 * (es_col >> 1) + (es_col & 1);
            asm volatile("" : "+v"(el0), "+v"(es0));
            auto efetch = [&](int kap, double (&f)[NNF ? NNF : 1], double (&g)[STRN ? STRN : 1]) {
#pragma unroll
                for (int nn = 0; nn < NNF; ++nn) f[nn] = LDS_UNPAIRED(eb[el0 + kap * 4 * A2P + 32 * nn]);
#pragma unroll
                for (int q = 0; q < STRN; ++q) g[q] = eb[es0 + kap * 4 * A2P + 8 * q];
            };
            double bf2[NNF ? NNF : 1], bs2[STRN ? STRN : 1];
            efetch(0, bf, bs);
            constexpr int KB2C = 4 * NQF + STRQ;
#pragma unroll
            for (int kap = 0; kap < KB2C; ++kap) {
                const int p = kap >> 2, t = kap & 3;
                double af2[MT];
#pragma unroll
                for (int m = 0; m < MT; ++m) af2[m] = p < NQF ? acc1[m][p < NQF ? p : 0][t] : acc1s[m][t < STRQ ? t : 0];
                if (kap & 1) {
                    if (kap + 1 < KB2C) efetch(kap + 1, bf, bs);
                    __builtin_amdgcn_sched_barrier(0);
#pragma unroll
                    for (int nn = 0; nn < NNF; ++nn)
#pragma unroll
                        for (int m = 0; m < MT; ++m) acc2[m][nn] = mfma16(af2[m], bf2[nn], acc2[m][nn]);
#pragma unroll
                    for (int q = 0; q < STRN; ++q)
#pragma unroll
                        for (int m = 0; m < MT; ++m) acc2s[m][q] = mfma4(af2[m], bs2[q], acc2s[m][q]);
                } else {
                    if (kap + 1 < KB2C) efetch(kap + 1, bf2, bs2);
                    __builtin_amdgcn_sched_barrier(0);
#pragma unroll
                    for (int nn = 0; nn < NNF; ++nn)
#pragma unroll
                        for (int m = 0; m < MT; ++m) acc2[m][nn] = mfma16(af2[m], bf[nn], acc2[m][nn]);
#pragma unroll
                    for (int q = 0; q < STRN; ++q)
#pragma unroll
                        for (int m = 0; m < MT; ++m) acc2s[m][q] = mfma4(af2[m], bs[q], acc2s[m][q]);
                }
            }
        }
        lds_barrier();
    }

    double *slab = a.slab + ((int64_t)prob * a.wpp * a.nac + unit) * a.J * a.A2;
#pragma unroll
    for (int m = 0; m < MT; ++m) {
#pragma unroll
        for (int nn = 0; nn < NNF; ++nn)
#pragma unroll
            for (int t = 0; t < 4; ++t) {
                const int j = j0[m] + 4 * t + kq, col = 16 * nn + x16;
                if (j < a.J && col < a.A2) slab[(int64_t)j * a.A2 + col] = acc2[m][nn][t];
            }
#pragma unroll
        for (int q = 0; q < STRN; ++q) {
            const int j = j0[m] + 4 * ((lane >> 2) & 3) + kq, col = 16 * NNF + 4 * q + (lane & 3);
            if (j < a.J && col < a.A2) slab[(int64_t)j * a.A2 + col] = acc2s[m][q];
        }
    }
}

template <int NQF, int STRQ, int NNF, int STRN, bool WT, int UNR, bool MT2>
__global__ __launch_bounds__(512, 2) void chain_wide_kernel(ChainWide a)
{
    extern __shared__ double cf_lds[];
    constexpr int AP = 16 * NQF + 4 * STRQ;
    double *Wl = cf_lds;
    double *El = cf_lds + a.ebase;
    const int tid = threadIdx.x, lane = tid & 63, w = tid >> 6;
    int prob, unit;
    chain_block_unit(a.xcd_map, a.wpp * a.nac, prob, unit);
    const int prob0 = prob * a.tpw;
    const int g = unit / a.nac, ac = unit - g * a.nac;
    const int a0 = ac * a.ac;
    const int cnt = a.A - a0 < a.ac ? a.A - a0 : a.ac;
    const int k_beg = (int)((int64_t)g * a.n / a.wpp), k_end = (int)((int64_t)(g + 1) * a.n / a.wpp);
    const int KB1 = ((a.K1 + 3) / 4 + UNR - 1) / UNR * UNR;
    const int A2P = a.A2P;

    for (int sl = 0; sl < a.tpw; ++sl) {
        if (prob0 + sl >= a.nb) break;
        const double *Wp = uniform_ptr(a.W[prob0 + sl]);
        double *Wd = Wl + (size_t)sl * a.wimg;
        const __amdgpu_buffer_rsrc_t rw = make_rsrc(Wp, ((int64_t)(a.K1 - 1) * a.w_c + a.A) * 8);
        const int total = 4 * KB1 * AP;
        constexpr int BATCH = 8;
        for (int e0 = tid; e0 < total; e0 += 512 * BATCH) {
            double v[BATCH];
#pragma unroll
            for (int u = 0; u < BATCH; ++u) {
                const int e = e0 + 512 * u;
                const int c = e / AP, col = e - c * AP;
                v[u] = ld8(rw, (e < total && c < a.K1 && col < cnt) ? (uint32_t)(((int64_t)c * a.w_c + a0 + col) * 8) : OOB_OFF, 0);
            }
#pragma unroll
            for (int u = 0; u < BATCH; ++u) {
                const int e = e0 + 512 * u;
                const int c = e / AP, col = e - c * AP;
                if (e < total) Wd[(c >> 1) * 2 * AP + 2 * col + (c & 1)] = v[u];
            }
        }
    }

    if (w == a.loader) {
        const int NI = a.eunits >> 6;
        const uint32_t inv = e_image_inv(A2P);
        const int64_t rowstride = (int64_t)a.n * a.A2;
        const int ebuf = a.eunits * 2;
        auto fill = [&](int k) {
            chain_e_fill_gather<true>(a, El + ((a.ebuf2 && (k & 1)) ? ebuf : 0), k, a0, A2P, inv, rowstride, NI, 0, 1, lane, AP);
        };
        __syncthreads();
        if (a.ebuf2) {
            if (k_beg < k_end) fill(k_beg);
            for (int k = k_beg; k < k_end; ++k) {
                asm volatile("s_waitcnt vmcnt(0)" ::: "memory");
                lds_barrier();
                if (k + 1 < k_end) fill(k + 1);
                lds_barrier();
            }
        } else {
            for (int k = k_beg; k < k_end; ++k) {
                fill(k);
                asm volatile("s_waitcnt vmcnt(0)" ::: "memory");
                lds_barrier();
                lds_barrier();
            }
        }
        return;
    }
    __syncthreads();
    const int t0 = a.tile0[w], t1 = a.tile1[w];
    const int myprob = prob0 + a.slot[w];
    if (t0 < 0 || myprob >= a.nb) return;
    const double *Wmine = Wl + (size_t)a.slot[w] * a.wimg;
    if constexpr (MT2) {
        if (t1 >= 0) {
            cw_compute<NQF, STRQ, NNF, STRN, WT, UNR, 2>(a, Wmine, El, myprob, unit, a0, cnt, k_beg, k_end, t0, t1);
            return;
        }
    }
    cw_compute<NQF, STRQ, NNF, STRN, WT, UNR, 1>(a, Wmine, El, myprob, unit, a0, cnt, k_beg, k_end, t0, -1);
}

int chain_wide_try(const ChainStepArgs &c, int stream, hipStream_t st, bool force = false);

}
```

### tt_sketch_amd/csrc/chain_wide.hip

```cpp
#include "chain_wide.h"
#include "prof.h"

namespace ttsk {

#define TTSK_CW_DECL(T) \
    int launch_chain_wide_##T(const ChainWide &a, int nn, int sn, bool wt, int unr, size_t lds, int grid, hipStream_t st);
TTSK_CW_DECL(0a) TTSK_CW_DECL(0b) TTSK_CW_DECL(1a) TTSK_CW_DECL(1b) TTSK_CW_DECL(2a) TTSK_CW_DECL(2b) TTSK_CW_DECL(3a)
TTSK_CW_DECL(3b) TTSK_CW_DECL(4a) TTSK_CW_DECL(4b) TTSK_CW_DECL(5a) TTSK_CW_DECL(5b) TTSK_CW_DECL(6a) TTSK_CW_DECL(6b)
#undef TTSK_CW_DECL

static int launch_chain_wide(int ci, const ChainWide &a, int nn, int sn, bool wt, int unr, size_t lds, int grid, hipStream_t st)
{
    const bool lo = nn <= 4;
    switch (ci) {
    case 0: return lo ? launch_chain_wide_0a(a, nn, sn, wt, unr, lds, grid, st) : launch_chain_wide_0b(a, nn, sn, wt, unr, lds, grid, st);
    case 1: return lo ? launch_chain_wide_1a(a, nn, sn, wt, unr, lds, grid, st) : launch_chain_wide_1b(a, nn, sn, wt, unr, lds, grid, st);
    case 2: return lo ? launch_chain_wide_2a(a, nn, sn, wt, unr, lds, grid, st) : launch_chain_wide_2b(a, nn, sn, wt, unr, lds, grid, st);
    case 3: return lo ? launch_chain_wide_3a(a, nn, sn, wt, unr, lds, grid, st) : launch_chain_wide_3b(a, nn, sn, wt, unr, lds, grid, st);
    case 4: return lo ? launch_chain_wide_4a(a, nn, sn, wt, unr, lds, grid, st) : launch_chain_wide_4b(a, nn, sn, wt, unr, lds, grid, st);
    case 5: return lo ? launch_chain_wide_5a(a, nn, sn, wt, unr, lds, grid, st) : launch_chain_wide_5b(a, nn, sn, wt, unr, lds, grid, st);
    default: return lo ? launch_chain_wide_6a(a, nn, sn, wt, unr, lds, grid, st) : launch_chain_wide_6b(a, nn, sn, wt, unr, lds, grid, st);
    }
}

int chain_wide_try(const ChainStepArgs &c, int stream, hipStream_t st, bool force)
{
    const int n_cu = device_num_cu();
    if (n_cu < 1) return TTSK_ERR_HIP;
    ChainWidePlan p;
    if (!chain_wide_plan(c, n_cu, force, p)) return 0;
    ChainWide &a = p.a;
    a.slab = chain_slab_request(stream, p.l);
    if (!a.slab) return TTSK_ERR_HIP;
    ProfBracket prof(st, PROF_CURRENT, p.l.flops,
                     "chain_wide_kernel<%d, %d, %d, %d, %s, %d, %s>", CW_NQ[p.ci], CW_SQ[p.ci], p.nn, p.sn, p.wt ? "true" : "false", p.unr,
                     p.mt2 ? "true" : "false");
    int rc = launch_chain_wide(p.ci, a, p.nn, p.sn, p.wt, p.unr, p.l.lds, p.l.grid, st);
    if (rc == TTSK_OK) rc = chain_slab_reduce(st, a.slab, p.l, c);
    return rc == TTSK_OK ? 1 : (rc == 1 ? 0 : rc);
}

}

using namespace ttsk;

extern "C" int ttsk_chain_step_wide(int nb, int n, int K1, int A, int A2, int J, const double *const *W, int64_t w_c,
                                    const double *const *X, int64_t x_j, int64_t x_k, int64_t x_c, int64_t x_extent,
                                    const double *E, double *const *T, double *const *Out, int stream)
{
    TTSK_STREAM(st, stream);
    TTSK_ARG(W && X && E && Out && nb >= 1, "ttsk_chain_step_wide: NULL argument");
    ChainStepArgs c{nb, n, K1, A, A2, J, W, w_c, X, x_j, x_k, x_c, x_extent, E, T, Out};
    const int rc = chain_wide_try(c, stream, st, true);
    if (rc == 0) {
        set_error("ttsk_chain_step_wide: shape (n=%d K1=%d A=%d A2=%d J=%d nb=%d) is not covered by the chunked fused kernel", n, K1,
                  A, A2, J, nb);
        return TTSK_ERR_UNSUPPORTED;
    }
    return rc < 0 ? rc : TTSK_OK;
}
```

### tt_sketch_amd/csrc/stream_small.h

```cpp
#pragma once
#include "skinny.h"
#include "psi_plan.h"

namespace ttsk {

template <int NF, int STR, int D, int UNR = 5 * D>
__global__ __launch_bounds__(512) void stream_small_kernel(StreamSmall a)
{
    static_assert(UNR % D == 0, "the unrolled body must keep the ring slots static");
    extern __shared__ double ss_lds[];
    double *Wl = ss_lds;
    const int tid = threadIdx.x, lane = tid & 63, w = tid >> 6;
    const int x16 = lane & 15, kq = lane >> 4;
    const int prob = blockIdx.x / (a.wpp * a.nac), unit = blockIdx.x - prob * (a.wpp * a.nac);
    const int g = unit / a.nac, a0 = (unit - g * a.nac) * a.ac;
    const int cnt = a.A - a0 < a.ac ? a.A - a0 : a.ac;
    const int KB1 = ((a.K1 + 3) / 4 + UNR - 1) / UNR * UNR, AP = a.AP;
    {
        const double *Wp = uniform_ptr(a.W[prob]);
        const __amdgpu_buffer_rsrc_t rw = make_rsrc(Wp, ((int64_t)(a.K1 - 1) * a.w_c + a.A) * 8);
        const int total = 4 * (KB1 + 1) * AP;
        constexpr int BATCH = 10;
        for (int e0 = tid; e0 < total; e0 += 512 * BATCH) {
            double v[BATCH];
#pragma unroll
            for (int u = 0; u < BATCH; ++u) {
                const int e = e0 + 512 * u;
                const int c = e / AP, col = e - c * AP;
                v[u] = ld8(rw, (e < total && c < a.K1 && col < cnt) ? (uint32_t)(((int64_t)c * a.w_c + a0 + col) * 8) : OOB_OFF, 0);
            }
#pragma unroll
            for (int u = 0; u < BATCH; ++u) {
                const int e = e0 + 512 * u;
                const int c = e / AP, col = e - c * AP;
                if (e < total) Wl[(c >> 1) * 2 * AP + 2 * col + (c & 1)] = v[u];
            }
        }
    }
    const int ntiles = (a.J + 15) >> 4;
    const int tstep = a.wpp * 8;
    int tile = g * 8 + w;
    const __amdgpu_buffer_rsrc_t rs = make_rsrc(uniform_ptr(a.S[prob]), a.s_extent * 8);
    const __amdgpu_buffer_rsrc_t rc = make_rsrc(uniform_ptr(a.C[prob]), a.c_extent * 8);
    const uint32_t slane = (uint32_t)(((int64_t)x16 * a.s_j + kq) * 8);
    const uint32_t tstride = __builtin_amdgcn_readfirstlane((uint32_t)(16 * a.s_j * 8));
    auto sload = [&](uint32_t so) -> double { return ld8(rs, slane, __builtin_amdgcn_readfirstlane(so)); };
    const int ITER = KB1 / UNR;
    double ring[D];
#pragma unroll
    for (int d = 0; d < D; ++d) ring[d] = sload((uint32_t)tile * tstride + (uint32_t)d * 32u);
    const int wl_lane = (kq >> 1) * 2 * AP + 2 * x16 + (kq & 1);
    const int ws_lane = (kq >> 1) * 2 * AP + 2 * (16 * NF + (x16 & 3)) + (kq & 1);
    __syncthreads();

    for (; tile < ntiles; tile += tstep) {
        v4d acc[NF ? NF : 1];
        double accs[STR ? STR : 1];
#pragma unroll
        for (int p = 0; p < NF; ++p)
#pragma unroll
            for (int t = 0; t < 4; ++t) acc[p][t] = 0.0;
#pragma unroll
        for (int q = 0; q < STR; ++q) accs[q] = 0.0;
        double bf[NF ? NF : 1], sf[STR ? STR : 1];
        auto wfetch = [&](const double *wrun, int u, double (&f)[NF ? NF : 1], double (&gq)[STR ? STR : 1]) {
#pragma unroll
            for (int p = 0; p < NF; ++p) f[p] = wrun[wl_lane + u * 4 * AP + 32 * p];
#pragma unroll
            for (int q = 0; q < STR; ++q) gq[q] = wrun[ws_lane + u * 4 * AP + 8 * q];
        };
        wfetch(Wl, 0, bf, sf);
        uint32_t so = (uint32_t)tile * tstride + (uint32_t)D * 32u;
        auto kblock = [&](const double *wrun, int u, bool wrap) {
            const int d = u % D;
            double bfn[NF ? NF : 1], sfn[STR ? STR : 1];
            wfetch(wrun, u + 1, bfn, sfn);
            const double af = ring[d];
#pragma unroll
            for (int p = 0; p < NF; ++p) acc[p] = mfma16(af, bf[p], acc[p]);
#pragma unroll
            for (int q = 0; q < STR; ++q) accs[q] = mfma4(af, sf[q], accs[q]);
            if (wrap) so = (uint32_t)(tile + tstep) * tstride;
            ring[d] = sload(so);
            so += 32u;
#pragma unroll
            for (int p = 0; p < NF; ++p) bf[p] = bfn[p];
#pragma unroll
            for (int q = 0; q < STR; ++q) sf[q] = sfn[q];
        };
        for (int it = 0; it < ITER; ++it) {
            const double *wrun = Wl + it * UNR * 4 * AP;
            const bool last = it == ITER - 1;
#pragma unroll
            for (int u = 0; u < UNR; ++u) kblock(wrun, u, last && u + D == UNR);
        }
        const int j0 = 16 * tile;
#pragma unroll
        for (int t = 0; t < 4; ++t) {
            const int j = j0 + 4 * t + kq;
            const uint32_t ro = (uint32_t)(((int64_t)j * a.c_j + a0 + x16) * 8);
#pragma unroll
            for (int p = 0; p < NF; ++p) {
                const uint32_t off = (j < a.J && 16 * p + x16 < cnt) ? ro + 128u * p : OOB_OFF;
                double v = acc[p][t];
                if (a.accumulate) v += ld8(rc, off, 0);
                st8(rc, off, v);
            }
        }
#pragma unroll
        for (int q = 0; q < STR; ++q) {
            const int j = j0 + 4 * ((lane >> 2) & 3) + kq, col = 16 * NF + 4 * q + (lane & 3);
            const uint32_t off = (j < a.J && col < cnt) ? (uint32_t)(((int64_t)j * a.c_j + a0 + col) * 8) : OOB_OFF;
            double v = accs[q];
            if (a.accumulate) v += ld8(rc, off, 0);
            st8(rc, off, v);
        }
    }
}

template <int NF, int STR, int D, int UNR = 5 * D>
__global__ __launch_bounds__(512) void stream_small_sum_kernel(StreamSmallSum a)
{
    static_assert(UNR % D == 0, "the unrolled body must keep the ring slots static");
    extern __shared__ double ss_lds[];
    const int tid = threadIdx.x, lane = tid & 63, w = tid >> 6;
    const int x16 = lane & 15, kq = lane >> 4;
    const int units = a.groups * a.nac;
    int unit = blockIdx.x;
    if (a.xcd_map) {
        const int upx = units >> 3, xcd = blockIdx.x & 7, j = blockIdx.x >> 3;
        unit = xcd * upx + j;
    }
    const int g = unit / a.nac, a0 = (unit - g * a.nac) * a.ac;
    const int cnt = a.A - a0 < a.ac ? a.A - a0 : a.ac;
    const int KB1 = ((a.K1 + 3) / 4 + UNR - 1) / UNR * UNR, AP = a.AP;
    const int img = 4 * (KB1 + 1) * AP;
    const __amdgpu_buffer_rsrc_t rw = make_rsrc(a.W, a.w_extent * 8);
    constexpr int BATCH = 12;
    double wv[BATCH];
    auto w_fetch = [&](int b) {
#pragma unroll
        for (int u = 0; u < BATCH; ++u) {
            const int e = tid + 512 * u;
            const int c = e / AP, col = e - c * AP;
            wv[u] = ld8(rw, (e < img && c < a.K1 && col < cnt) ? (uint32_t)(((int64_t)b * a.w_b + (int64_t)c * a.w_c + a0 + col) * 8) : OOB_OFF, 0);
        }
    };
    auto w_store = [&](double *Wl) {
#pragma unroll
        for (int u = 0; u < BATCH; ++u) {
            const int e = tid + 512 * u;
            const int c = e / AP, col = e - c * AP;
            if (e < img) Wl[(c >> 1) * 2 * AP + 2 * col + (c & 1)] = wv[u];
        }
    };
    w_fetch(0);
    w_store(ss_lds);
    const int ntiles = (a.J + 15) >> 4;
    const int tile = g * 8 + w;
    const bool live = tile < ntiles;
    const __amdgpu_buffer_rsrc_t rs = make_rsrc(a.S, a.s_extent * 8);
    const __amdgpu_buffer_rsrc_t rc = make_rsrc(a.C, a.c_extent * 8);
    const uint32_t slane = live ? (uint32_t)((((int64_t)tile * 16 + x16) * a.s_j + kq) * 8) : OOB_OFF;
    const uint32_t bstride = __builtin_amdgcn_readfirstlane((uint32_t)(a.s_b * 8));
    auto sload = [&](uint32_t so) -> double { return ld8(rs, slane, __builtin_amdgcn_readfirstlane(so)); };
    const int ITER = KB1 / UNR;
    double ring[D];
#pragma unroll
    for (int d = 0; d < D; ++d) ring[d] = sload((uint32_t)d * 32u);
    const int wl_lane = (kq >> 1) * 2 * AP + 2 * x16 + (kq & 1);
    const int ws_lane = (kq >> 1) * 2 * AP + 2 * (16 * NF + (x16 & 3)) + (kq & 1);
    v4d acc[NF ? NF : 1];
    double accs[STR ? STR : 1];
#pragma unroll
    for (int p = 0; p < NF; ++p)
#pragma unroll
        for (int t = 0; t < 4; ++t) acc[p][t] = 0.0;
#pragma unroll
    for (int q = 0; q < STR; ++q) accs[q] = 0.0;
    __syncthreads();
    for (int b = 0; b < a.nb; ++b) {
        const double *Wl = ss_lds + (size_t)(b & 1) * img;
        if (b + 1 < a.nb) w_fetch(b + 1);
        double bf[NF ? NF : 1], sf[STR ? STR : 1];
        auto wfetch = [&](const double *wrun, int u, double (&f)[NF ? NF : 1], double (&gq)[STR ? STR : 1]) {
#pragma unroll
            for (int p = 0; p < NF; ++p) f[p] = wrun[wl_lane + u * 4 * AP + 32 * p];
#pragma unroll
            for (int q = 0; q < STR; ++q) gq[q] = wrun[ws_lane + u * 4 * AP + 8 * q];
        };
        wfetch(Wl, 0, bf, sf);
        uint32_t so = (uint32_t)b * bstride + (uint32_t)D * 32u;
        auto kblock = [&](const double *wrun, int u, bool wrap) {
            const int d = u % D;
            double bfn[NF ? NF : 1], sfn[STR ? STR : 1];
            wfetch(wrun, u + 1, bfn, sfn);
            const double af = ring[d];
#pragma unroll
            for (int p = 0; p < NF; ++p) acc[p] = mfma16(af, bf[p], acc[p]);
#pragma unroll
            for (int q = 0; q < STR; ++q) accs[q] = mfma4(af, sf[q], accs[q]);
            if (wrap) so = (uint32_t)(b + 1) * bstride;
            ring[d] = sload(so);
            so += 32u;
#pragma unroll
            for (int p = 0; p < NF; ++p) bf[p] = bfn[p];
#pragma unroll
            for (int q = 0; q < STR; ++q) sf[q] = sfn[q];
        };
        for (int it = 0; it < ITER; ++it) {
            const double *wrun = Wl + it * UNR * 4 * AP;
            const bool last = it == ITER - 1;
#pragma unroll
            for (int u = 0; u < UNR; ++u) kblock(wrun, u, last && u + D == UNR);
        }
        if (b + 1 < a.nb) w_store(ss_lds + (size_t)((b + 1) & 1) * img);
        __syncthreads();
    }
    if (!live) return;
    const int j0 = 16 * tile;
#pragma unroll
    for (int t = 0; t < 4; ++t) {
        const int j = j0 + 4 * t + kq;
        const uint32_t ro = (uint32_t)(((int64_t)j * a.c_j + a0 + x16) * 8);
#pragma unroll
        for (int p = 0; p < NF; ++p) {
            const uint32_t off = (j < a.J && 16 * p + x16 < cnt) ? ro + 128u * p : OOB_OFF;
            double v = acc[p][t];
            if (a.accumulate) v += ld8(rc, off, 0);
            st8(rc, off, v);
        }
    }
#pragma unroll
    for (int q = 0; q < STR; ++q) {
        const int j = j0 + 4 * ((lane >> 2) & 3) + kq, col = 16 * NF + 4 * q + (lane & 3);
        const uint32_t off = (j < a.J && col < cnt) ? (uint32_t)(((int64_t)j * a.c_j + a0 + col) * 8) : OOB_OFF;
        double v = accs[q];
        if (a.accumulate) v += ld8(rc, off, 0);
        st8(rc, off, v);
    }
}

int stream_small_sum_try(const StreamSmallSumArgs &c, int stream, hipStream_t st);
int stream_small_try(const StreamSmallArgs &c, int stream, hipStream_t st);

}
```

### tt_sketch_amd/csrc/stream_small.hip

```cpp
#include <cstdlib>
#include "stream_small.h"
#include "prof.h"

namespace ttsk {

static int launch_ss(const StreamSmall &a, int nf, int str, int unr, size_t lds, int grid, hipStream_t st)
{
#define TTSK_SS_CASE(NF, STR) if (nf == NF && str == STR) return launch(unr == 25 ? stream_small_kernel<NF, STR, 5, 25> : stream_small_kernel<NF, STR, 5, 5>, dim3((unsigned)grid), dim3(512), lds, st, a);
    PSI_STREAM_STRUCTURES(TTSK_SS_CASE)
#undef TTSK_SS_CASE
    return 1;
}

int stream_small_try(const StreamSmallArgs &c, int stream, hipStream_t st)
{
    (void)stream;
    PsiStreamPlan p;
    const int ok = psi_stream_plan(c, device_num_cu(), p);
    if (ok != 1) return ok;
    ProfBracket prof(st, PROF_CURRENT, p.l.flops, "%s", p.l.name);
    const int rc = launch_ss(p.a, p.nf, p.str, p.unr, p.l.lds, p.l.grid, st);
    return rc == TTSK_OK ? 1 : (rc == 1 ? 0 : rc);
}

static int launch_sss(const StreamSmallSum &a, int nf, int str, int unr, size_t lds, int grid, hipStream_t st)
{
#define TTSK_SSS_CASE(NF, STR) if (nf == NF && str == STR) return launch(unr == 25 ? stream_small_sum_kernel<NF, STR, 5, 25> : stream_small_sum_kernel<NF, STR, 5, 5>, dim3((unsigned)grid), dim3(512), lds, st, a);
    PSI_STREAM_SUM_STRUCTURES(TTSK_SSS_CASE)
#undef TTSK_SSS_CASE
    return 1;
}

int stream_small_sum_try(const StreamSmallSumArgs &c, int stream, hipStream_t st)
{
    (void)stream;
    PsiStreamSumPlan p;
    const int ok = psi_stream_sum_plan(c, device_num_cu(), p);
    if (ok != 1) return ok;
    ProfBracket prof(st, PROF_CURRENT, p.l.flops, "%s", p.l.name);
    const int rc = launch_sss(p.a, p.nf, p.str, p.unr, p.l.lds, p.l.grid, st);
    return rc == TTSK_OK ? 1 : (rc == 1 ? 0 : rc);
}

}

using namespace ttsk;

extern "C" int ttsk_psi_stream(int nb, int J, int K1, int A, const double *const *S, int64_t s_j, const double *const *W,
                               int64_t w_c, double *const *C, int64_t c_j, int accumulate, int stream)
{
    TTSK_STREAM(st, stream);
    TTSK_ARG(S && W && C, "ttsk_psi_stream: NULL argument");
    for (int b = 0; b < nb && b < SK_MAXB; ++b) TTSK_ARG(S[b] && W[b] && C[b], "ttsk_psi_stream: NULL operand of problem %d", b);
    const StreamSmallArgs c{nb, J, K1, A, S, s_j, W, w_c, C, c_j, accumulate};
    const int rc = stream_small_try(c, stream, st);
    if (rc == 0) {
        set_error("ttsk_psi_stream: shape (nb=%d J=%d K1=%d A=%d s_j=%lld w_c=%lld c_j=%lld) is not covered by the streamed kernel", nb, J, K1,
                  A, (long long)s_j, (long long)w_c, (long long)c_j);
        return TTSK_ERR_UNSUPPORTED;
    }
    return rc < 0 ? rc : TTSK_OK;
}

extern "C" int ttsk_psi_stream_sum(int nb, int J, int K1, int A, const double *S, int64_t s_j, int64_t s_b, const double *W,
                                   int64_t w_c, int64_t w_b, double *C, int64_t c_j, int accumulate, int stream)
{
    TTSK_STREAM(st, stream);
    TTSK_ARG(S && W && C, "ttsk_psi_stream_sum: NULL argument");
    const StreamSmallSumArgs c{nb, J, K1, A, S, s_j, s_b, W, w_c, w_b, C, c_j, accumulate};
    const int rc = stream_small_sum_try(c, stream, st);
    if (rc == 0) {
        set_error("ttsk_psi_stream_sum: shape (nb=%d J=%d K1=%d A=%d s_j=%lld s_b=%lld w_c=%lld w_b=%lld c_j=%lld) is not covered by the "
                  "summing streamed kernel", nb, J, K1, A, (long long)s_j, (long long)s_b, (long long)w_c, (long long)w_b, (long long)c_j);
        return TTSK_ERR_UNSUPPORTED;
    }
    return rc < 0 ? rc : TTSK_OK;
}
```

### tt_sketch_amd/csrc/tt_fused.hip

```cpp
#include <algorithm>
#include <cstdlib>
#include <vector>
#include "common.h"
#include "prof.h"
#include "skinny.h"
#include "chain_fused.h"
#include "chain_wide.h"
#include "chain_sum.h"
#include "tt_chain.h"
#include "stream_small.h"

namespace ttsk {

static int gemm(int cls, const ttsk_gemm_desc &d, const double *A, const double *B, double *C, int stream)
{
    ProfClass pc(cls);
    return ttsk_gemm(&d, A, B, C, nullptr, stream);
}

struct BatchPtrs {
    const double *A[SK_MAXB], *B[SK_MAXB];
    double *C[SK_MAXB];
};

static int gemm_batch(int cls, int nb, ttsk_gemm_desc d, const BatchPtrs &p, int stream, hipStream_t st,
                      bool chain_only = false)
{
    ProfClass pc(cls);
    ttsk_gemm_desc n = d;
    if (n.Ki == 1) { n.Ki = n.Ko; n.Ko = 1; n.a_ki = n.a_ko; n.b_ki = n.b_ko; }
    else if (n.Ko > 1 && n.a_ko == n.Ki * n.a_ki && n.b_ko == n.Ki * n.b_ki) { n.Ki *= n.Ko; n.Ko = 1; }
    int rc = skinny_try_batch(n, nb, p.A, p.B, p.C, stream, st);
    if (rc == 0 && !chain_only) rc = small_try_batch(n, nb, p.A, p.B, p.C, stream, st);
    if (rc == 0 && !chain_only) {
        rc = 1;
        for (int b = 0; b < nb && rc == 1; ++b) {
            const int e = ttsk_gemm(&d, p.A[b], p.B[b], p.C[b], nullptr, stream);
            if (e != TTSK_OK) rc = e;
        }
    }
    return rc;
}

template <class Args>
static int psi_stream(int (*try_launch)(const Args &, int, hipStream_t), Args a, int64_t J, int q, hipStream_t st)
{
    if (J >= (1ll << 30)) return 0;
    a.J = (int)J;
    ProfClass pc(4);
    return try_launch(a, q, st);
}

static int64_t sketch_offsets(int d, const int64_t *n, const int64_t *l_lo, const int64_t *l_hi, const int64_t *r_lo,
                              const int64_t *r_hi, size_t *psi_at = nullptr, size_t *om_at = nullptr)
{
    int64_t tot = 0;
    for (int mu = 0; mu < d; ++mu) {
        int64_t l = mu == 0 ? 1 : l_hi[mu - 1] - l_lo[mu - 1];
        int64_t r = mu == d - 1 ? 1 : r_hi[d - 2 - mu] - r_lo[d - 2 - mu];
        if (psi_at) psi_at[mu] = tot;
        tot += l * n[mu] * r;
    }
    for (int mu = 0; mu < d - 1; ++mu) {
        if (om_at) om_at[mu] = tot;
        tot += (l_hi[mu] - l_lo[mu]) * (r_hi[d - 2 - mu] - r_lo[d - 2 - mu]);
    }
    return tot;
}

struct SketchWs {
    int nb, d;
    const int64_t *n, *s, *lt, *l_lo, *l_hi, *rt, *r_lo, *r_hi;
    bool sum;
    std::vector<size_t> offL, offR, offT, szL, szR, szT;
    size_t offTR, szTR, offP0, szP0, offPs, szPs, bytes;
    std::vector<size_t> psi_at, om_at;
    std::vector<int> t_inter;
    double *ws0 = nullptr;

    static size_t even(size_t v) { return v + (v & 1); }
    static size_t blk(size_t v) { return (v + 31) & ~(size_t)31; }
    int64_t lw(int mu) const { return l_hi[mu] - l_lo[mu]; }
    int64_t rw(int j) const { return r_hi[j] - r_lo[j]; }

    SketchWs(int nb_, int d_, const int64_t *n_, const int64_t *s_, const int64_t *lt_, const int64_t *l_lo_, const int64_t *l_hi_,
             const int64_t *rt_, const int64_t *r_lo_, const int64_t *r_hi_, bool sum_)
        : nb(nb_), d(d_), n(n_), s(s_), lt(lt_), l_lo(l_lo_), l_hi(l_hi_), rt(rt_), r_lo(r_lo_), r_hi(r_hi_), sum(sum_), offL(d - 1),
          offR(d - 1), offT(d), szL(d - 1), szR(d - 1), szT(d), psi_at(d), om_at(d - 1), t_inter(d, 0)
    {
        size_t tot = 0;
        for (int mu = 0; mu < d - 1; ++mu) { szL[mu] = even((size_t)s[mu + 1] * lt[mu + 1]); offL[mu] = tot; tot += blk(nb * szL[mu]); }
        for (int j = 0; j < d - 1; ++j) { szR[j] = even((size_t)s[d - 1 - j] * rt[j + 1]); offR[j] = tot; tot += blk(nb * szR[j]); }
        for (int mu = 1; mu < d; ++mu) { szT[mu] = even((size_t)lt[mu] * n[mu] * s[mu + 1]); offT[mu] = tot; tot += blk(nb * szT[mu]); }
        size_t tr_max = 0;
        for (int mu = 1; mu < d - 1; ++mu) tr_max = std::max(tr_max, (size_t)rt[d - 1 - mu] * n[mu] * s[mu]);
        szTR = even(tr_max), offTR = tot;
        tot += blk(nb * szTR);
        szP0 = even((size_t)n[0] * rw(d - 2)), offP0 = tot;
        if (sum) tot += blk(nb * szP0);
        szPs = 0;
        for (int mu = 1; sum && mu < d - 1; ++mu) szPs = std::max(szPs, even((size_t)lw(mu - 1) * n[mu] * rw(d - 2 - mu)));
        offPs = tot;
        tot += 2 * blk(nb * szPs);
        bytes = tot * 8;
        sketch_offsets(d, n, l_lo, l_hi, r_lo, r_hi, psi_at.data(), om_at.data());
    }

    double *Lp(int b, int mu) const { return ws0 + offL[mu] + (size_t)b * szL[mu]; }
    double *Rp(int b, int j) const { return ws0 + offR[j] + (size_t)b * szR[j]; }
    double *Tp0(int b, int mu) const { return ws0 + offT[mu] + (size_t)b * szT[mu]; }
    double *TRp(int b) const { return ws0 + offTR + (size_t)b * szTR; }
    double *P0(int b) const { return ws0 + offP0 + (size_t)b * szP0; }
    double *Ps(int half) const { return ws0 + offPs + (size_t)half * blk(nb * szPs); }
    bool packedL(int mu) const { return szL[mu] == (size_t)s[mu + 1] * lt[mu + 1]; }
    bool packedR(int j) const { return szR[j] == (size_t)s[d - 1 - j] * rt[j + 1]; }
    const double *Lslice(int b, int mu) const { return Lp(b, mu) + l_lo[mu]; }
    const double *Rslice(int b, int j) const { return Rp(b, j) + r_lo[j]; }
    int64_t t_ld(int mu) const { return t_inter[mu] ? (int64_t)nb * s[mu + 1] : s[mu + 1]; }
    const double *Tslice(int b, int mu) const
    {
        const size_t row0 = (size_t)(l_lo[mu - 1] * n[mu]);
        return t_inter[mu] ? ws0 + offT[mu] + row0 * t_ld(mu) + (size_t)b * s[mu + 1] : Tp0(b, mu) + row0 * s[mu + 1];
    }
};

struct Ctx : SketchWs {
    const double *const *X, *const *DL, *const *DR;
    double *out;
    int64_t out_stride;
    int accumulate, stream;
    hipStream_t st;
    bool keep_t;
    int aux = 0; hipStream_t st_aux = nullptr;
    const double *Xc(int b, int mu) const { return X[(size_t)b * d + mu]; }
    double *outb(int b) const { return out + (size_t)b * out_stride; }
};

#define CK(x) do { rc = (x); if (rc < 0) return rc; } while (0)

static int check_ranks(const char *who, int d, const int64_t *s, const int64_t *lt, const int64_t *l_lo, const int64_t *l_hi,
                       const int64_t *rt, const int64_t *r_lo, const int64_t *r_hi)
{
    TTSK_ARG(s[0] == 1 && s[d] == 1 && lt[0] == 1 && rt[0] == 1, "%s: boundary ranks must be 1", who);
    for (int mu = 0; mu < d - 1; ++mu) {
        TTSK_ARG(0 <= l_lo[mu] && l_lo[mu] <= l_hi[mu] && l_hi[mu] <= lt[mu + 1], "%s: left rank slice %d out of range", who, mu);
        TTSK_ARG(0 <= r_lo[mu] && r_lo[mu] <= r_hi[mu] && r_hi[mu] <= rt[mu + 1], "%s: right rank slice %d out of range", who, mu);
    }
    return TTSK_OK;
}

static int chain_step_try(int cls, const ChainSumArgs &ca, int stream, hipStream_t st)
{
    const ChainStepArgs &cs = ca.s;
    ProfClass pc(cls);
    int fz = (cs.K1 <= 128 && cs.J <= 128 && cs.A <= 128 && cs.A2 <= 128) ? chain_fused_try(cs, stream, st) : 0;
    if (fz == 0 && (fz = chain_sum_try(ca, stream, st)) == 1) return 2;
    if (fz == 0) fz = chain_wide_try(cs, stream, st);
    return fz;
}

static int right_step(const Ctx &c, int j)
{
    const int nb = c.nb, mu = c.d - 1 - j;
    const int64_t sp = c.s[mu + 1], sn = c.s[mu], nn = c.n[mu], rho = c.rt[j], rhop = c.rt[j + 1];
    int rc;
    BatchPtrs p{};
    if (j == 0) {
        for (int b = 0; b < nb; ++b) { p.A[b] = c.Xc(b, mu); p.B[b] = c.DR[j]; p.C[b] = c.Rp(b, j); }
        CK(gemm_batch(5, nb, gemm_desc2(sn, rhop, 1, nn, nn * sp, 0, sp, 0, rhop, 1, rhop, 1, 0), p, c.stream, c.st));
        return TTSK_OK;
    }
    for (int b = 0; b < nb; ++b) { p.A[b] = c.Rp(b, j - 1); p.B[b] = c.Xc(b, mu); p.C[b] = c.Rp(b, j); }
    const ChainStepArgs cs{nb, (int)nn, (int)sp, (int)rho, (int)rhop, (int)sn, p.A, rho, p.B, nn * sp, sp, 1, sn * nn * sp,
                           c.DR[j], nullptr, p.C};
    CK(chain_step_try(1, ChainSumArgs{cs, nullptr, 0, 0, 0}, c.stream, c.st));
    if (rc) return TTSK_OK;
    const bool merged = nb > 1 && c.packedR(j) && (int64_t)nb * sn * rho * nn <= (int64_t)nb * c.szTR;
    const int64_t ldt = merged ? (int64_t)nb * sn : sn;
    for (int b = 0; b < nb; ++b) { p.A[b] = c.Rp(b, j - 1); p.B[b] = c.Xc(b, mu); p.C[b] = merged ? c.TRp(0) + (size_t)b * sn : c.TRp(b); }
    ttsk_gemm_desc g1 = gemm_desc2(rho, sn, 1, sp, 1, 0, rho, 0, 1, nn * sp, nn * ldt, 1, 0);
    g1.batch = nn; g1.b_b = sp; g1.c_b = ldt;
    const int fast = gemm_batch(0, nb, g1, p, c.stream, c.st, !merged);
    if (fast < 0) return fast;
    BatchPtrs q{};
    if (merged) {
        q.A[0] = c.TRp(0); q.B[0] = c.DR[j]; q.C[0] = c.Rp(0, j);
        CK(gemm_batch(1, 1, gemm_desc2((int64_t)nb * sn, rhop, rho, nn, 1, nn * ldt, ldt, nn * rhop, rhop, 1, rhop, 1, 0), q,
                      c.stream, c.st));
        return TTSK_OK;
    }
    for (int b = 0; b < nb; ++b) { q.A[b] = c.TRp(b); q.B[b] = c.DR[j]; q.C[b] = c.Rp(b, j); }
    if (fast == 1) {
        CK(gemm_batch(1, nb, gemm_desc2(sn, rhop, rho, nn, 1, nn * sn, sn, nn * rhop, rhop, 1, rhop, 1, 0), q, c.stream, c.st));
    } else {
        CK(gemm_batch(0, nb, gemm_desc2(rho, sn * nn, 1, sp, 1, 0, rho, 0, 1, sp, sn * nn, 1, 0), p, c.stream, c.st));
        CK(gemm_batch(1, nb, gemm_desc2(sn, rhop, rho, nn, nn, sn * nn, 1, nn * rhop, rhop, 1, rhop, 1, 0), q, c.stream, c.st));
    }
    return TTSK_OK;
}

static int left_step(Ctx &c, int mu)
{
    const int nb = c.nb, d = c.d;
    const int64_t sn = c.s[mu], sp = c.s[mu + 1], nn = c.n[mu], *lt = c.lt;
    int rc;
    BatchPtrs p{};
    if (mu == 0) {
        for (int b = 0; b < nb; ++b) { p.A[b] = c.Xc(b, 0); p.B[b] = c.DL[0]; p.C[b] = c.Lp(b, 0); }
        CK(gemm_batch(5, nb, gemm_desc2(sp, lt[1], 1, nn, 1, 0, sp, 0, lt[1], 1, lt[1], 1, 0), p, c.aux, c.st_aux));
        return TTSK_OK;
    }
    const int64_t lfull = lt[mu];
    if (mu < d - 1) {
        double *Tp[SK_MAXB];
        for (int b = 0; b < nb; ++b) { p.A[b] = c.Lp(b, mu - 1); p.B[b] = c.Xc(b, mu); p.C[b] = c.Lp(b, mu); Tp[b] = c.Tp0(b, mu); }
        const ChainStepArgs cs{nb, (int)nn, (int)sn, (int)lfull, (int)lt[mu + 1], (int)sp, p.A, lfull, p.B, 1, sp, nn * sp,
                               sn * nn * sp, c.DL[mu], c.keep_t ? Tp : nullptr, p.C};
        const bool inter = c.sum && nb > 1 && c.packedL(mu);
        const ChainSumArgs ca = c.keep_t ? ChainSumArgs{cs, c.Tp0(0, mu), inter ? sp : (int64_t)c.szT[mu], inter ? (int64_t)nb * sp : sp,
                                                        (int64_t)nb * (int64_t)c.szT[mu]}
                                         : ChainSumArgs{cs, nullptr, 0, 0, 0};
        CK(chain_step_try(3, ca, c.aux, c.st_aux));
        if (rc == 2 && inter) c.t_inter[mu] = 1;
        if (rc) return TTSK_OK;
    }
    const bool merged = nb > 1 && mu < d - 1 && c.packedL(mu);
    if (merged) {
        c.t_inter[mu] = 1;
        const int64_t ldt = (int64_t)nb * sp;
        double *T0 = c.Tp0(0, mu);
        for (int b = 0; b < nb; ++b) { p.A[b] = c.Lp(b, mu - 1); p.B[b] = c.Xc(b, mu); p.C[b] = T0 + (size_t)b * sp; }
        ttsk_gemm_desc g1 = gemm_desc2(lfull, sp, 1, sn, 1, 0, lfull, 0, nn * sp, 1, nn * ldt, 1, 0);
        g1.batch = nn; g1.b_b = sp; g1.c_b = ldt;
        CK(gemm_batch(2, nb, g1, p, c.aux, c.st_aux));
        BatchPtrs q{};
        q.A[0] = T0; q.B[0] = c.DL[mu]; q.C[0] = c.Lp(0, mu);
        CK(gemm_batch(3, 1, gemm_desc2((int64_t)nb * sp, lt[mu + 1], lfull, nn, 1, nn * ldt, ldt, nn * lt[mu + 1], lt[mu + 1], 1,
                                  lt[mu + 1], 1, 0), q, c.aux, c.st_aux));
        return TTSK_OK;
    }
    if (mu == d - 1 && !c.sum) {
        if (c.lw(mu - 1) == 0) return TTSK_OK;
        for (int b = 0; b < nb; ++b) { p.A[b] = c.Lslice(b, mu - 1); p.B[b] = c.Xc(b, mu); p.C[b] = c.outb(b) + c.psi_at[mu]; }
        CK(gemm_batch(5, nb, gemm_desc2(c.lw(mu - 1), nn * sp, 1, sn, 1, 0, lfull, 0, nn * sp, 1, nn * sp, 1, c.accumulate), p, c.aux,
                      c.st_aux));
        return TTSK_OK;
    }
    for (int b = 0; b < nb; ++b) { p.A[b] = c.Lp(b, mu - 1); p.B[b] = c.Xc(b, mu); p.C[b] = c.Tp0(b, mu); }
    CK(gemm_batch(mu == d - 1 ? 5 : 2, nb, gemm_desc2(lfull, nn * sp, 1, sn, 1, 0, lfull, 0, nn * sp, 1, nn * sp, 1, 0), p,
                  c.aux, c.st_aux));
    if (mu < d - 1) {
        BatchPtrs q{};
        for (int b = 0; b < nb; ++b) { q.A[b] = c.Tp0(b, mu); q.B[b] = c.DL[mu]; q.C[b] = c.Lp(b, mu); }
        CK(gemm_batch(3, nb, gemm_desc2(sp, lt[mu + 1], 1, lfull * nn, 1, 0, sp, 0, lt[mu + 1], 1, lt[mu + 1], 1, 0), q,
                      c.aux, c.st_aux));
    }
    return TTSK_OK;
}

static int run_chains(Ctx &c, bool left)
{
    const char *single = getenv("TTSK_SINGLE_STREAM");
    c.aux = (single && single[0] == '1') ? c.stream : (c.stream + 1) % TTSK_NUM_STREAMS;
    if (!(c.st_aux = stream_of(c.aux))) return TTSK_ERR_ARG;
    if (!(c.ws0 = (double *)scratch(c.stream, SCRATCH_DRIVER, c.bytes))) return TTSK_ERR_HIP;
    int rc;
    CK(ttsk_stream_wait(c.aux, c.stream));
    for (int t = 0; t < c.d; ++t) {
        if (t < c.d - 1) CK(right_step(c, t));
        if (left && (t < c.d - 1 || c.keep_t)) CK(left_step(c, t));
    }
    return TTSK_OK;
}

constexpr int sum_psi_split = 48;

static int psi_sum_one_product(const Ctx &c, int mu, int q)
{
    const int nb = c.nb, jr = c.d - 2 - mu;
    const int64_t sp = c.s[mu + 1], nn = c.n[mu], l = c.lw(mu - 1), r = c.rw(jr), ldr = c.rt[jr + 1], ldt = c.t_ld(mu);
    double *psi = c.out + c.psi_at[mu];
    int rc;
    const bool one_index = c.t_inter[mu] && c.packedR(jr);
    if (one_index && l * nn >= 1024) {
        const int64_t K = (int64_t)nb * sp;
        const int nch = stream_small_chunks(K, r, nb);
        if (nch >= 1) {
            const int64_t Kc = K / nch;
            double *blk0 = c.Ps(mu & 1);
            BatchPtrs p{};
            for (int cidx = 0; cidx < nch; ++cidx) {
                p.A[cidx] = c.Tslice(0, mu) + (size_t)cidx * Kc; p.B[cidx] = c.Rslice(0, jr) + (size_t)cidx * Kc * ldr;
                p.C[cidx] = nch == 1 ? psi : blk0 + (size_t)cidx * c.szPs;
            }
            const StreamSmallArgs ss{nch, 0 , (int)Kc, (int)r, p.A, ldt, p.B, ldr, p.C, r, nch == 1 ? c.accumulate : 0};
            CK(psi_stream(stream_small_try, ss, l * nn, q, stream_of(q)));
            if (rc == 1) return nch > 1 ? ttsk_sum_slices(psi, blk0, nch, c.szPs, (size_t)(l * nn * r), c.accumulate, q) : TTSK_OK;
        }
    }
    return gemm(4, one_index ? gemm_desc2(l * nn, r, 1, (int64_t)nb * sp, ldt, 0, 1, 0, ldr, 1, r, 1, c.accumulate)
                             : gemm_desc2(l * nn, r, nb, sp, ldt, c.t_inter[mu] ? sp : (int64_t)c.szT[mu], 1, (int64_t)c.szR[jr], ldr, 1,
                                     r, 1, c.accumulate), c.Tslice(0, mu), c.Rslice(0, jr), psi, q);
}

static int psi_omega(const Ctx &c, int mu, int q, bool do_psi, bool do_omega)
{
    const int nb = c.nb, d = c.d;
    const int64_t sp = c.s[mu + 1], nn = c.n[mu];
    hipStream_t stq = stream_of(q);
    const int jr = d - 2 - mu;
    const int64_t ldr = mu < d - 1 ? c.rt[jr + 1] : 0, r = mu < d - 1 ? c.rw(jr) : 1;
    int rc = 0;
    BatchPtrs p{};
    if (!do_psi) {
    } else if (mu == 0) {
        for (int b = 0; b < nb; ++b) { p.A[b] = c.Xc(b, 0); p.B[b] = c.Rslice(b, jr); p.C[b] = c.sum ? c.P0(b) : c.outb(b) + c.psi_at[0]; }
        CK(gemm_batch(5, nb, gemm_desc2(nn, r, 1, sp, sp, 0, 1, 0, ldr, 1, r, 1, c.sum ? 0 : c.accumulate), p, q, stq));
        if (c.sum) CK(ttsk_sum_slices(c.out + c.psi_at[0], c.P0(0), nb, c.szP0, (size_t)(nn * r), c.accumulate, q));
    } else if (mu == d - 1) {
        if (c.sum) CK(ttsk_sum_slices(c.out + c.psi_at[mu], c.Tslice(0, mu), nb, c.szT[mu], (size_t)(c.lw(mu - 1) * nn), c.accumulate, q));
    } else if (c.sum && sp <= sum_psi_split) {
        CK(psi_sum_one_product(c, mu, q));
    } else {
        const int64_t l = c.lw(mu - 1), ldt = c.t_ld(mu);
        if (c.sum && !c.t_inter[mu]) {
            const size_t t_len = (size_t)c.lt[mu] * nn * sp;
            if (c.szT[mu] != t_len)
                TTSK_HIP(hipMemset2DAsync(c.Tp0(0, mu) + t_len, c.szT[mu] * 8, 0, 8, (size_t)nb, stq));
            const StreamSmallSumArgs sa{nb, 0 , (int)sp, (int)r, c.Tslice(0, mu), ldt, (int64_t)c.szT[mu],
                                        c.Rslice(0, jr), ldr, (int64_t)c.szR[jr], c.out + c.psi_at[mu], r, c.accumulate};
            CK(psi_stream(stream_small_sum_try, sa, l * nn, q, stq));
        }
        if (rc == 0) {
            double *blk0 = c.Ps(mu & 1);
            for (int b = 0; b < nb; ++b) {
                p.A[b] = c.Tslice(b, mu); p.B[b] = c.Rslice(b, jr); p.C[b] = c.sum ? blk0 + (size_t)b * c.szPs : c.outb(b) + c.psi_at[mu];
            }
            const int acc = c.sum ? 0 : c.accumulate;
            const StreamSmallArgs ss{nb, 0 , (int)sp, (int)r, p.A, ldt, p.B, ldr, p.C, r, acc};
            CK(psi_stream(stream_small_try, ss, l * nn, q, stq));
            if (rc == 0) CK(gemm_batch(4, nb, gemm_desc2(l * nn, r, 1, sp, ldt, 0, 1, 0, ldr, 1, r, 1, acc), p, q, stq));
            if (c.sum) CK(ttsk_sum_slices(c.out + c.psi_at[mu], blk0, nb, c.szPs, (size_t)(l * nn * r), c.accumulate, q));
        }
    }
    if (mu == d - 1 || !do_omega) return TTSK_OK;
    const int64_t l = c.lw(mu);
    if (c.sum)
        return gemm(5, c.packedL(mu) && c.packedR(jr)
                           ? gemm_desc2(l, r, 1, (int64_t)nb * sp, 1, 0, c.lt[mu + 1], 0, ldr, 1, r, 1, c.accumulate)
                           : gemm_desc2(l, r, nb, sp, 1, (int64_t)c.szL[mu], c.lt[mu + 1], (int64_t)c.szR[jr], ldr, 1, r, 1, c.accumulate),
                    c.Lslice(0, mu), c.Rslice(0, jr), c.out + c.om_at[mu], q);
    ttsk_gemm_desc od = gemm_desc2(l, r, 1, sp, 1, 0, c.lt[mu + 1], 0, ldr, 1, r, 1, c.accumulate);
    od.batch = nb; od.a_b = (int64_t)c.szL[mu]; od.b_b = (int64_t)c.szR[jr]; od.c_b = c.out_stride;
    return gemm(5, od, c.Lslice(0, mu), c.Rslice(0, jr), c.outb(0) + c.om_at[mu], q);
}

static int tail_grouped(const Ctx &c, bool ends_early)
{
    const int nb = c.nb, d = c.d;
    if (c.sum || d < 4 || nb * (d - 1) > SK_MAXB) return 0;
    bool psis_and_omegas_one_shape = c.s[d - 1] == c.s[1] && c.lw(d - 2) == c.lw(0) && c.lt[d - 1] == c.lt[1] && c.rw(d - 2) == c.rw(0) &&
                                     c.rt[d - 1] == c.rt[1];
    for (int mu = 1; mu < d - 1; ++mu)
        psis_and_omegas_one_shape = psis_and_omegas_one_shape && c.n[mu] == c.n[1] && c.s[mu] == c.s[1] && c.s[mu + 1] == c.s[1] &&
                                    c.t_inter[mu] == c.t_inter[1] && c.lw(mu - 1) == c.lw(0) && c.lt[mu] == c.lt[1] &&
                                    c.lt[mu + 1] == c.lt[1] && c.rw(d - 2 - mu) == c.rw(0) && c.rt[d - 1 - mu] == c.rt[1];
    if (!psis_and_omegas_one_shape) return 0;
    const int64_t sp = c.s[1], nn = c.n[1], l = c.lw(0), r = c.rw(0), ldr = c.rt[1];
    int rc;
    BatchPtrs p{};
    int cnt = 0;
    for (int mu = 1; mu < d - 1; ++mu)
        for (int b = 0; b < nb; ++b, ++cnt) {
            p.A[cnt] = c.Tslice(b, mu); p.B[cnt] = c.Rslice(b, d - 2 - mu); p.C[cnt] = c.outb(b) + c.psi_at[mu];
        }
    const StreamSmallArgs ss{cnt, 0 , (int)sp, (int)r, p.A, c.t_ld(1), p.B, ldr, p.C, r, c.accumulate};
    CK(psi_stream(stream_small_try, ss, l * nn, c.stream, c.st));
    if (rc == 0) return 0;
    BatchPtrs o{};
    cnt = 0;
    for (int mu = 0; mu < d - 1; ++mu)
        for (int b = 0; b < nb; ++b, ++cnt) {
            o.A[cnt] = c.Lslice(b, mu); o.B[cnt] = c.Rslice(b, d - 2 - mu); o.C[cnt] = c.outb(b) + c.om_at[mu];
        }
    CK(gemm_batch(5, cnt, gemm_desc2(l, r, 1, sp, 1, 0, c.lt[1], 0, ldr, 1, r, 1, c.accumulate), o, c.aux, c.st_aux));
    if (!ends_early) CK(psi_omega(c, 0, c.aux, true, false));
    CK(psi_omega(c, d - 1, c.stream, true, false));
    return 1;
}

static int tail_sum(const Ctx &c, bool &om_batched, bool &psi_batched)
{
    const int nb = c.nb, d = c.d;
    int rc;
    bool omegas_one_packed_shape = d - 1 <= SK_MAXB && d >= 3;
    for (int mu = 0; mu < d - 1 && omegas_one_packed_shape; ++mu)
        omegas_one_packed_shape = c.s[mu + 1] == c.s[1] && c.lt[mu + 1] == c.lt[1] && c.rt[d - 1 - mu] == c.rt[d - 1] && c.packedL(mu) &&
                                  c.packedR(d - 2 - mu) && c.lw(mu) == c.lw(0) && c.rw(d - 2 - mu) == c.rw(d - 2);
    if (omegas_one_packed_shape) {
        BatchPtrs o{};
        for (int mu = 0; mu < d - 1; ++mu) { o.A[mu] = c.Lslice(0, mu); o.B[mu] = c.Rslice(0, d - 2 - mu); o.C[mu] = c.out + c.om_at[mu]; }
        const int64_t l = c.lw(0), r = c.rw(d - 2);
        CK(gemm_batch(5, d - 1, gemm_desc2(l, r, 1, (int64_t)nb * c.s[1], 1, 0, c.lt[1], 0, c.rt[d - 1], 1, r, 1, c.accumulate), o, c.aux, c.st_aux));
        om_batched = true;
    }
    if (d < 4) return TTSK_OK;
    const int64_t sp = c.s[2], nn = c.n[1], l = c.lw(0), r = c.rw(d - 3), ldr = c.rt[d - 2];
    bool psis_one_interleaved_shape = l * nn >= 1024;
    for (int mu = 1; mu < d - 1 && psis_one_interleaved_shape; ++mu) {
        const int jr = d - 2 - mu;
        psis_one_interleaved_shape = c.t_inter[mu] && c.packedR(jr) && c.n[mu] == nn && c.s[mu + 1] == sp && c.lw(mu - 1) == l &&
                                     c.rw(jr) == r && c.rt[jr + 1] == ldr;
    }
    if (!psis_one_interleaved_shape) return TTSK_OK;
    const int64_t K = (int64_t)nb * sp;
    const int nch = stream_small_chunks(K, r, nb);
    if (!(nch > 1 && (d - 2) * nch <= SK_MAXB && (d - 2) * nch <= 2 * nb && c.szPs >= (size_t)(l * nn * r))) return TTSK_OK;
    const int64_t Kc = K / nch, ldt = (int64_t)nb * sp;
    double *blk0 = c.Ps(0);
    BatchPtrs p{};
    int cnt = 0;
    for (int mu = 1; mu < d - 1; ++mu) {
        const double *T0 = c.Tslice(0, mu), *R0 = c.Rslice(0, d - 2 - mu);
        for (int cidx = 0; cidx < nch; ++cidx, ++cnt) {
            p.A[cnt] = T0 + (size_t)cidx * Kc; p.B[cnt] = R0 + (size_t)cidx * Kc * ldr; p.C[cnt] = blk0 + (size_t)cnt * c.szPs;
        }
    }
    const StreamSmallArgs ss{cnt, 0 , (int)Kc, (int)r, p.A, ldt, p.B, ldr, p.C, r, 0};
    CK(psi_stream(stream_small_try, ss, l * nn, c.stream, c.st));
    if (rc == 0) return TTSK_OK;
    psi_batched = true;
    CK(ttsk_stream_wait(c.aux, c.stream));
    for (int mu = 1; mu < d - 1; ++mu)
        CK(ttsk_sum_slices(c.out + c.psi_at[mu], blk0 + (size_t)(mu - 1) * nch * c.szPs, nch, c.szPs, (size_t)(l * nn * r),
                           c.accumulate, (mu & 1) ? c.aux : c.stream));
    return TTSK_OK;
}

}

using namespace ttsk;

extern "C" {

int64_t ttsk_tt_sketch_size(int d, const int64_t *n, const int64_t *l_lo, const int64_t *l_hi,
                            const int64_t *r_lo, const int64_t *r_hi)
{
    return sketch_offsets(d, n, l_lo, l_hi, r_lo, r_hi);
}

int ttsk_tt_sketch(int d, const int64_t *n, const int64_t *s, const int64_t *lt, const int64_t *l_lo,
                   const int64_t *l_hi, const int64_t *rt, const int64_t *r_lo, const int64_t *r_hi,
                   const double *const *X, const double *const *DL, const double *const *DR, double *out,
                   int accumulate, int stream)
{
    return ttsk_tt_sketch_batch(1, d, n, s, lt, l_lo, l_hi, rt, r_lo, r_hi, X, DL, DR, out, 0, accumulate, stream);
}

static int tt_sketch_core(int nb, int d, const int64_t *n, const int64_t *s, const int64_t *lt, const int64_t *l_lo,
                          const int64_t *l_hi, const int64_t *rt, const int64_t *r_lo, const int64_t *r_hi,
                          const double *const *X, const double *const *DL, const double *const *DR, double *out,
                          int64_t out_stride, int accumulate, int stream, bool sum)
{
    TTSK_STREAM(st, stream);
    TTSK_ARG(nb >= 1, "ttsk_tt_sketch_batch: need nb >= 1, got %d", nb);
    TTSK_ARG(d >= 2, "ttsk_tt_sketch: need d >= 2, got %d", d);
    TTSK_ARG(n && s && lt && l_lo && l_hi && rt && r_lo && r_hi && X && DR && DL && out, "ttsk_tt_sketch: NULL argument");
    int rc;
    CK(check_ranks("ttsk_tt_sketch", d, s, lt, l_lo, l_hi, rt, r_lo, r_hi));
    const int64_t one = ttsk_tt_sketch_size(d, n, l_lo, l_hi, r_lo, r_hi);
    TTSK_ARG(sum || nb == 1 || out_stride >= one, "ttsk_tt_sketch_batch: out_stride %lld < sketch size %lld",
             (long long)out_stride, (long long)one);
    if (nb > SK_MAXB) {
        for (int b0 = 0; b0 < nb; b0 += SK_MAXB) {
            const int cnt = nb - b0 < SK_MAXB ? nb - b0 : SK_MAXB;
            rc = tt_sketch_core(cnt, d, n, s, lt, l_lo, l_hi, rt, r_lo, r_hi, X + (size_t)b0 * d, DL, DR,
                                sum ? out : out + (size_t)b0 * out_stride, out_stride, (sum && b0) ? 1 : accumulate,
                                stream, sum);
            if (rc) return rc;
        }
        return TTSK_OK;
    }
    if (nb == 1) sum = false;
    Ctx c{SketchWs(nb, d, n, s, lt, l_lo, l_hi, rt, r_lo, r_hi, sum), X, DL, DR, out, out_stride, accumulate, stream, st, true};
    CK(run_chains(c, true));
    const bool ends_early = !sum && d >= 3;
    if (ends_early) CK(psi_omega(c, 0, stream, true, false));
    CK(ttsk_stream_wait(stream, c.aux));
    CK(ttsk_stream_wait(c.aux, stream));
    CK(tail_grouped(c, ends_early));
    if (rc == 0) {
        bool om_batched = false, psi_batched = false;
        if (sum) CK(tail_sum(c, om_batched, psi_batched));
        for (int mu = 0; mu < d; ++mu) {
            const bool psi_here = !(psi_batched && mu >= 1 && mu < d - 1) && !(ends_early && mu == 0);
            if (!psi_here && (om_batched || mu == d - 1)) continue;
            CK(psi_omega(c, mu, (mu & 1) ? c.aux : stream, psi_here, !om_batched));
        }
    }
    CK(ttsk_stream_wait(stream, c.aux));
    return TTSK_OK;
}

int ttsk_tt_sketch_batch(int nb, int d, const int64_t *n, const int64_t *s, const int64_t *lt, const int64_t *l_lo,
                         const int64_t *l_hi, const int64_t *rt, const int64_t *r_lo, const int64_t *r_hi,
                         const double *const *X, const double *const *DL, const double *const *DR, double *out,
                         int64_t out_stride, int accumulate, int stream)
{
    return tt_sketch_core(nb, d, n, s, lt, l_lo, l_hi, rt, r_lo, r_hi, X, DL, DR, out, out_stride, accumulate, stream, false);
}

int ttsk_tt_sketch_sum(int nb, int d, const int64_t *n, const int64_t *s, const int64_t *lt, const int64_t *l_lo,
                       const int64_t *l_hi, const int64_t *rt, const int64_t *r_lo, const int64_t *r_hi,
                       const double *const *X, const double *const *DL, const double *const *DR, double *out,
                       int accumulate, int stream)
{
    return tt_sketch_core(nb, d, n, s, lt, l_lo, l_hi, rt, r_lo, r_hi, X, DL, DR, out, 0, accumulate, stream, true);
}

}

namespace ttsk {

int tt_chains(int d, const int64_t *n, const int64_t *s, const int64_t *lt, const int64_t *rt, const double *const *X,
              const double *const *DL, const double *const *DR, TTChains *out, int stream)
{
    return tt_chains_batch(1, d, n, s, lt, rt, X, DL, DR, out, stream);
}

int tt_chains_batch(int nb, int d, const int64_t *n, const int64_t *s, const int64_t *lt, const int64_t *rt, const double *const *X,
                    const double *const *DL, const double *const *DR, TTChains *out, int stream)
{
    if (d < 2 || d > 64 || !out) { set_error("tt_chains: bad argument"); return TTSK_ERR_ARG; }
    const bool left = out->want_left;
    std::vector<int64_t> zero(d, 0), lhi(d, 1), rhi(d, 1), ones(d + 1, 1);
    for (int mu = 0; mu < d - 1; ++mu) rhi[mu] = rt[mu + 1];
    for (int mu = 0; left && mu < d - 1; ++mu) lhi[mu] = lt[mu + 1];
    if (nb < 1 || nb > SK_MAXB) { set_error("tt_chains: %d tensors (1 .. %d)", nb, SK_MAXB); return TTSK_ERR_ARG; }
    TTSK_STREAM(st, stream);
    const int64_t *lt_ = left ? lt : ones.data();
    TTSK_ARG(n && s && lt_ && rt && X && DR && (DL || !left), "tt_chains: NULL argument");
    int rc;
    CK(check_ranks("tt_chains", d, s, lt_, zero.data(), lhi.data(), rt, zero.data(), rhi.data()));
    Ctx c{SketchWs(nb, d, n, s, lt_, zero.data(), lhi.data(), rt, zero.data(), rhi.data(), false), X, DL, DR, nullptr, 0, 0, stream,
          st, false};
    CK(run_chains(c, left));
    for (int j = 0; j < d - 1; ++j) { out->Rc[j] = c.Rp(0, j); out->r_stride[j] = (int64_t)c.szR[j]; }
    for (int mu = 0; mu < d - 1; ++mu) { out->Lc[mu] = left ? c.Lp(0, mu) : nullptr; out->l_stride[mu] = (int64_t)c.szL[mu]; }
    if (!left) return TTSK_OK;
    CK(ttsk_stream_wait(stream, c.aux));
    bool chain_pairs_one_shape = true;
    for (int mu = 1; mu < d - 1; ++mu)
        chain_pairs_one_shape = chain_pairs_one_shape && s[mu + 1] == s[1] && lt[mu + 1] == lt[1] && rt[d - 1 - mu] == rt[d - 1];
    BatchPtrs o{};
    int cnt = 0;
    for (int b = 0; b < nb; ++b)
        for (int mu = 0; mu < d - 1; ++mu) {
            o.A[cnt] = c.Lp(b, mu); o.B[cnt] = c.Rp(b, d - 2 - mu); o.C[cnt] = out->omega[(size_t)b * (d - 1) + mu];
            if (chain_pairs_one_shape && ++cnt < SK_MAXB && !(b == nb - 1 && mu == d - 2)) continue;
            const int64_t l = lt[mu + 1], r = rt[d - 1 - mu];
            CK(gemm_batch(5, chain_pairs_one_shape ? cnt : 1, gemm_desc2(l, r, 1, s[mu + 1], 1, 0, l, 0, r, 1, r, 1, 0), o, stream, st));
            cnt = 0;
        }
    return TTSK_OK;
}

#undef CK

}
```

Baseline: 58920.

## Partition CUs between concurrent right and left chain kernels in pipelined sketches

Adds a CU-budget policy that, when sketches are pipelined across two streams and all chain steps use the fused kernel, splits the compute units between the right-chain and left-chain kernels in proportion to their estimated flops. Each kernel planner then sizes its grid for the reduced budget, so the two concurrent launches do not compete for the same CUs. A public API lets the caller override the budgets. The policy relies on a heuristic work estimate and may leave CUs idle if the split is unbalanced; it also removes one error message on chain_sum launch failure.

```diff
diff --git a/include/ttsk.h b/include/ttsk.h
--- a/include/ttsk.h
+++ b/include/ttsk.h
@@ -66,6 +66,7 @@
                        const int64_t *l_hi, const int64_t *rt, const int64_t *r_lo, const int64_t *r_hi,
                        const double *const *X, const double *const *DL, const double *const *DR,
                        double *out, int accumulate, int stream);
+int ttsk_tt_sketch_split(int right_cus, int left_cus, int psi_cus);
 int ttsk_chain_step(int nb, int n, int K1, int A, int A2, int J, const double *const *W, int64_t w_c,
                     const double *const *X, int64_t x_j, int64_t x_k, int64_t x_c, int64_t x_extent,
                     const double *E, double *const *T, double *const *Out, int stream);
diff --git a/tt_sketch_amd/_native.py b/tt_sketch_amd/_native.py
--- a/tt_sketch_amd/_native.py
+++ b/tt_sketch_amd/_native.py
@@ -81,6 +81,7 @@
     "ttsk_tt_sketch": Entry([I] + [POINTER(I64)] * 8 + [POINTER(P)] * 3 + [P, I, I], FORK_NEXT),
     "ttsk_tt_sketch_batch": Entry([I, I] + [POINTER(I64)] * 8 + [POINTER(P)] * 3 + [P, I64, I, I], FORK_NEXT),
     "ttsk_tt_sketch_sum": Entry([I, I] + [POINTER(I64)] * 8 + [POINTER(P)] * 3 + [P, I, I], FORK_NEXT),
+    "ttsk_tt_sketch_split": Entry([I, I, I]),
     "ttsk_chain_step": Entry(_CHAIN + [POINTER(P), POINTER(P), I], QUEUE),
     "ttsk_chain_step_wide": Entry(_CHAIN + [POINTER(P), POINTER(P), I], QUEUE),
     "ttsk_chain_step_sum": Entry(_CHAIN + [P, I64, I64, I64, POINTER(P), I], QUEUE),
diff --git a/tt_sketch_amd/csrc/chain_fused.h b/tt_sketch_amd/csrc/chain_fused.h
--- a/tt_sketch_amd/csrc/chain_fused.h
+++ b/tt_sketch_amd/csrc/chain_fused.h
@@ -408,7 +408,7 @@
     return launch_r_reduce(st, slab, r);
 }
 
-int chain_fused_try(const ChainStepArgs &c, int stream, hipStream_t st, bool force = false);
+int chain_fused_try(const ChainStepArgs &c, int stream, hipStream_t st, bool force = false, int cus = 0);
 
 const double *drm_packed_lookup(const double *E, int A, int n, int A2, int A2P, int eunits);
 
diff --git a/tt_sketch_amd/csrc/chain_fused.hip b/tt_sketch_amd/csrc/chain_fused.hip
--- a/tt_sketch_amd/csrc/chain_fused.hip
+++ b/tt_sketch_amd/csrc/chain_fused.hip
@@ -19,12 +19,12 @@
     return launch_chain_step_e(a, nf, str, wt, ebuf, unr, waves, lds, grid, st);
 }
 
-int chain_fused_try(const ChainStepArgs &c, int stream, hipStream_t st, bool force)
+int chain_fused_try(const ChainStepArgs &c, int stream, hipStream_t st, bool force, int cus)
 {
     const int n_cu = device_num_cu();
     if (n_cu < 1) return TTSK_ERR_HIP;
     ChainFusedPlan p;
-    if (!chain_fused_plan(c, n_cu, force, p)) return 0;
+    if (!chain_fused_plan(c, cus > 0 ? cus : n_cu, force, p)) return 0;
     ChainStep &a = p.a;
     a.slab = chain_slab_request(stream, p.l);
     if (!a.slab) return TTSK_ERR_HIP;
diff --git a/tt_sketch_amd/csrc/chain_sum.h b/tt_sketch_amd/csrc/chain_sum.h
--- a/tt_sketch_amd/csrc/chain_sum.h
+++ b/tt_sketch_amd/csrc/chain_sum.h
@@ -466,7 +466,7 @@
 #endif
 }
 
-int chain_sum_try(const ChainSumArgs &c, int stream, hipStream_t st, bool force = false);
+int chain_sum_try(const ChainSumArgs &c, int stream, hipStream_t st, bool force = false, int cus = 0);
 int launch_chain_sum_2(const ChainSum &a, bool wt, size_t lds, int grid, hipStream_t st);
 int launch_chain_sum_4(const ChainSum &a, bool wt, size_t lds, int grid, hipStream_t st);
 
diff --git a/tt_sketch_amd/csrc/chain_sum.hip b/tt_sketch_amd/csrc/chain_sum.hip
--- a/tt_sketch_amd/csrc/chain_sum.hip
+++ b/tt_sketch_amd/csrc/chain_sum.hip
@@ -4,13 +4,13 @@
 
 namespace ttsk {
 
-int chain_sum_try(const ChainSumArgs &cc, int stream, hipStream_t st, bool force)
+int chain_sum_try(const ChainSumArgs &cc, int stream, hipStream_t st, bool force, int cus)
 {
     const ChainStepArgs &c = cc.s;
     const int n_cu = device_num_cu();
     if (n_cu < 1) return TTSK_ERR_HIP;
     ChainSumPlan p;
-    if (!chain_sum_plan(cc, n_cu, force, p)) return 0;
+    if (!chain_sum_plan(cc, cus > 0 ? cus : n_cu, force, p)) return 0;
     ChainSum &ka = p.ka;
     ChainSumS &a = ka.s;
     a.slab = chain_slab_request(stream, p.l);
@@ -28,7 +28,6 @@
     }
 #endif
     int rc = p.na_run <= 2 ? launch_chain_sum_2(ka, p.wt, p.l.lds, p.l.grid, st) : launch_chain_sum_4(ka, p.wt, p.l.lds, p.l.grid, st);
-    if (rc != TTSK_OK) set_error("chain_sum_kernel launch failed");
 #ifdef TTSK_LAB
     if (stamps_on) {
         long long h[8 * 8 * 8];
diff --git a/tt_sketch_amd/csrc/chain_wide.h b/tt_sketch_amd/csrc/chain_wide.h
--- a/tt_sketch_amd/csrc/chain_wide.h
+++ b/tt_sketch_amd/csrc/chain_wide.h
@@ -272,6 +272,6 @@
     cw_compute<NQF, STRQ, NNF, STRN, WT, UNR, 1>(a, Wmine, El, myprob, unit, a0, cnt, k_beg, k_end, t0, -1);
 }
 
-int chain_wide_try(const ChainStepArgs &c, int stream, hipStream_t st, bool force = false);
+int chain_wide_try(const ChainStepArgs &c, int stream, hipStream_t st, bool force = false, int cus = 0);
 
 }
diff --git a/tt_sketch_amd/csrc/chain_wide.hip b/tt_sketch_amd/csrc/chain_wide.hip
--- a/tt_sketch_amd/csrc/chain_wide.hip
+++ b/tt_sketch_amd/csrc/chain_wide.hip
@@ -23,12 +23,12 @@
     }
 }
 
-int chain_wide_try(const ChainStepArgs &c, int stream, hipStream_t st, bool force)
+int chain_wide_try(const ChainStepArgs &c, int stream, hipStream_t st, bool force, int cus)
 {
     const int n_cu = device_num_cu();
     if (n_cu < 1) return TTSK_ERR_HIP;
     ChainWidePlan p;
-    if (!chain_wide_plan(c, n_cu, force, p)) return 0;
+    if (!chain_wide_plan(c, cus > 0 ? cus : n_cu, force, p)) return 0;
     ChainWide &a = p.a;
     a.slab = chain_slab_request(stream, p.l);
     if (!a.slab) return TTSK_ERR_HIP;
diff --git a/tt_sketch_amd/csrc/sketch_split.h b/tt_sketch_amd/csrc/sketch_split.h
--- /dev/null
+++ b/tt_sketch_amd/csrc/sketch_split.h
@@ -0,0 +1,62 @@
+#pragma once
+#include <cstdint>
+
+namespace ttsk {
+
+struct SketchSplit {
+    int right, left, psi;
+};
+
+enum SketchFamily { SKETCH_FUSED = 0, SKETCH_OTHER = 1 };
+
+struct SketchSplitIn {
+    int n_cu, nb, d;
+    const int64_t *n;
+    const int64_t *s, *lt, *rt;
+    bool two_streams;
+    bool pipelined;
+    SketchFamily family;
+};
+
+constexpr int SPLIT_MIN_NB = 8;
+constexpr int SPLIT_MIN_WPP = 3;
+
+constexpr SketchSplit SKETCH_SPLIT_FULL{0, 0, 0};
+
+inline void sketch_chain_work(const SketchSplitIn &in, double &right, double &left)
+{
+    right = left = 0;
+    for (int mu = 1; mu < in.d - 1; ++mu) {
+        const int j = in.d - 1 - mu;
+        const double n = (double)in.n[mu], sn = (double)in.s[mu], sp = (double)in.s[mu + 1];
+        right += n * sn * (sp * in.rt[j] + (double)in.rt[j] * in.rt[j + 1]);
+        left += n * sp * (sn * in.lt[mu] + (double)in.lt[mu] * in.lt[mu + 1]);
+    }
+}
+
+inline SketchSplit sketch_split_policy(const SketchSplitIn &in)
+{
+    if (!in.two_streams || !in.pipelined || in.family != SKETCH_FUSED) return SKETCH_SPLIT_FULL;
+    if (in.nb < SPLIT_MIN_NB || in.n_cu < 1 || in.d < 3) return SKETCH_SPLIT_FULL;
+    int wpp = in.n_cu / in.nb;
+    for (int mu = 1; mu < in.d - 1; ++mu)
+        if (in.n[mu] < wpp) wpp = (int)in.n[mu];
+    if (wpp < SPLIT_MIN_WPP) return SKETCH_SPLIT_FULL;
+    double wr_flops, wl_flops;
+    sketch_chain_work(in, wr_flops, wl_flops);
+    if (!(wr_flops > 0) || !(wl_flops > 0)) return SKETCH_SPLIT_FULL;
+    const int share = wpp - 1;
+    int wr = (int)((double)share * wr_flops / (wr_flops + wl_flops) + 0.5);
+    if (wr > share - 1) wr = share - 1;
+    if (wr < 1) wr = 1;
+    return SketchSplit{wr * in.nb, (share - wr) * in.nb, 0};
+}
+
+inline SketchSplit sketch_split_resolve(const SketchSplitIn &in, const int set[3])
+{
+    const SketchSplit pol = (set[0] < 0 || set[1] < 0 || set[2] < 0) ? sketch_split_policy(in) : SKETCH_SPLIT_FULL;
+    auto pick = [&](int s, int p) { return s < 0 ? p : (s > in.n_cu ? in.n_cu : s); };
+    return SketchSplit{pick(set[0], pol.right), pick(set[1], pol.left), pick(set[2], pol.psi)};
+}
+
+}
diff --git a/tt_sketch_amd/csrc/stream_small.h b/tt_sketch_amd/csrc/stream_small.h
--- a/tt_sketch_amd/csrc/stream_small.h
+++ b/tt_sketch_amd/csrc/stream_small.h
@@ -241,7 +241,7 @@
     }
 }
 
-int stream_small_sum_try(const StreamSmallSumArgs &c, int stream, hipStream_t st);
-int stream_small_try(const StreamSmallArgs &c, int stream, hipStream_t st);
+int stream_small_sum_try(const StreamSmallSumArgs &c, int stream, hipStream_t st, int cus = 0);
+int stream_small_try(const StreamSmallArgs &c, int stream, hipStream_t st, int cus = 0);
 
 }
diff --git a/tt_sketch_amd/csrc/stream_small.hip b/tt_sketch_amd/csrc/stream_small.hip
--- a/tt_sketch_amd/csrc/stream_small.hip
+++ b/tt_sketch_amd/csrc/stream_small.hip
@@ -12,11 +12,11 @@
     return 1;
 }
 
-int stream_small_try(const StreamSmallArgs &c, int stream, hipStream_t st)
+int stream_small_try(const StreamSmallArgs &c, int stream, hipStream_t st, int cus)
 {
     (void)stream;
     PsiStreamPlan p;
-    const int ok = psi_stream_plan(c, device_num_cu(), p);
+    const int ok = psi_stream_plan(c, cus > 0 ? cus : device_num_cu(), p);
     if (ok != 1) return ok;
     ProfBracket prof(st, PROF_CURRENT, p.l.flops, "%s", p.l.name);
     const int rc = launch_ss(p.a, p.nf, p.str, p.unr, p.l.lds, p.l.grid, st);
@@ -31,11 +31,11 @@
     return 1;
 }
 
-int stream_small_sum_try(const StreamSmallSumArgs &c, int stream, hipStream_t st)
+int stream_small_sum_try(const StreamSmallSumArgs &c, int stream, hipStream_t st, int cus)
 {
     (void)stream;
     PsiStreamSumPlan p;
-    const int ok = psi_stream_sum_plan(c, device_num_cu(), p);
+    const int ok = psi_stream_sum_plan(c, cus > 0 ? cus : device_num_cu(), p);
     if (ok != 1) return ok;
     ProfBracket prof(st, PROF_CURRENT, p.l.flops, "%s", p.l.name);
     const int rc = launch_sss(p.a, p.nf, p.str, p.unr, p.l.lds, p.l.grid, st);
diff --git a/tt_sketch_amd/csrc/tt_fused.hip b/tt_sketch_amd/csrc/tt_fused.hip
--- a/tt_sketch_amd/csrc/tt_fused.hip
+++ b/tt_sketch_amd/csrc/tt_fused.hip
@@ -1,4 +1,5 @@
 #include <algorithm>
+#include <atomic>
 #include <cstdlib>
 #include <vector>
 #include "common.h"
@@ -9,6 +10,7 @@
 #include "chain_sum.h"
 #include "tt_chain.h"
 #include "stream_small.h"
+#include "sketch_split.h"
 
 namespace ttsk {
 
@@ -43,13 +45,16 @@
 }
 
 template <class Args>
-static int psi_stream(int (*try_launch)(const Args &, int, hipStream_t), Args a, int64_t J, int q, hipStream_t st)
+static int psi_stream(int (*try_launch)(const Args &, int, hipStream_t, int), Args a, int64_t J, int q, hipStream_t st, int cus)
 {
     if (J >= (1ll << 30)) return 0;
     a.J = (int)J;
     ProfClass pc(4);
-    return try_launch(a, q, st);
-}
+    return try_launch(a, q, st, cus);
+}
+
+static std::atomic<int> split_set[3] = {{-1}, {-1}, {-1}};
+static std::atomic<int> last_sketch_stream{-1};
 
 static int64_t sketch_offsets(int d, const int64_t *n, const int64_t *l_lo, const int64_t *l_hi, const int64_t *r_lo,
                               const int64_t *r_hi, size_t *psi_at = nullptr, size_t *om_at = nullptr)
@@ -132,6 +137,7 @@
     hipStream_t st;
     bool keep_t;
     int aux = 0; hipStream_t st_aux = nullptr;
+    SketchSplit cus = SKETCH_SPLIT_FULL;
     const double *Xc(int b, int mu) const { return X[(size_t)b * d + mu]; }
     double *outb(int b) const { return out + (size_t)b * out_stride; }
 };
@@ -149,13 +155,24 @@
     return TTSK_OK;
 }
 
-static int chain_step_try(int cls, const ChainSumArgs &ca, int stream, hipStream_t st)
+static bool chain_step_fits_fused(int64_t K1, int64_t J, int64_t A, int64_t A2) { return K1 <= 128 && J <= 128 && A <= 128 && A2 <= 128; }
+
+static bool step_on_fused(int64_t K1, int64_t J, int64_t A, int64_t A2)
+{
+    if (!chain_step_fits_fused(K1, J, A, A2) || J > 112 || A < 4 || A2 < 4 || (A2 & 1) || 2 * K1 < A) return false;
+    int nq, sq, nn, sn;
+    chain_tile_split((int)A, nq, sq);
+    chain_tile_split((int)A2, nn, sn);
+    return nq == nn && sq == sn && nq >= 1 && nq + (sq ? 1 : 0) <= 7;
+}
+
+static int chain_step_try(int cls, const ChainSumArgs &ca, int stream, hipStream_t st, int cus)
 {
     const ChainStepArgs &cs = ca.s;
     ProfClass pc(cls);
-    int fz = (cs.K1 <= 128 && cs.J <= 128 && cs.A <= 128 && cs.A2 <= 128) ? chain_fused_try(cs, stream, st) : 0;
+    int fz = chain_step_fits_fused(cs.K1, cs.J, cs.A, cs.A2) ? chain_fused_try(cs, stream, st, false, cus) : 0;
     if (fz == 0 && (fz = chain_sum_try(ca, stream, st)) == 1) return 2;
-    if (fz == 0) fz = chain_wide_try(cs, stream, st);
+    if (fz == 0) fz = chain_wide_try(cs, stream, st, false, cus);
     return fz;
 }
 
@@ -173,7 +190,7 @@
     for (int b = 0; b < nb; ++b) { p.A[b] = c.Rp(b, j - 1); p.B[b] = c.Xc(b, mu); p.C[b] = c.Rp(b, j); }
     const ChainStepArgs cs{nb, (int)nn, (int)sp, (int)rho, (int)rhop, (int)sn, p.A, rho, p.B, nn * sp, sp, 1, sn * nn * sp,
                            c.DR[j], nullptr, p.C};
-    CK(chain_step_try(1, ChainSumArgs{cs, nullptr, 0, 0, 0}, c.stream, c.st));
+    CK(chain_step_try(1, ChainSumArgs{cs, nullptr, 0, 0, 0}, c.stream, c.st, c.cus.right));
     if (rc) return TTSK_OK;
     const bool merged = nb > 1 && c.packedR(j) && (int64_t)nb * sn * rho * nn <= (int64_t)nb * c.szTR;
     const int64_t ldt = merged ? (int64_t)nb * sn : sn;
@@ -220,7 +237,7 @@
         const ChainSumArgs ca = c.keep_t ? ChainSumArgs{cs, c.Tp0(0, mu), inter ? sp : (int64_t)c.szT[mu], inter ? (int64_t)nb * sp : sp,
                                                         (int64_t)nb * (int64_t)c.szT[mu]}
                                          : ChainSumArgs{cs, nullptr, 0, 0, 0};
-        CK(chain_step_try(3, ca, c.aux, c.st_aux));
+        CK(chain_step_try(3, ca, c.aux, c.st_aux, c.cus.left));
         if (rc == 2 && inter) c.t_inter[mu] = 1;
         if (rc) return TTSK_OK;
     }
@@ -262,6 +279,19 @@
 {
     const char *single = getenv("TTSK_SINGLE_STREAM");
     c.aux = (single && single[0] == '1') ? c.stream : (c.stream + 1) % TTSK_NUM_STREAMS;
+    const int n_cu = device_num_cu();
+    if (n_cu < 1) return TTSK_ERR_HIP;
+    bool fused = true;
+    for (int mu = 1; mu < c.d - 1 && fused; ++mu) {
+        const int j = c.d - 1 - mu;
+        fused = step_on_fused(c.s[mu + 1], c.s[mu], c.rt[j], c.rt[j + 1]) && (!left || step_on_fused(c.s[mu], c.s[mu + 1], c.lt[mu], c.lt[mu + 1]));
+    }
+    const int set[3] = {split_set[0].load(), split_set[1].load(), split_set[2].load()};
+    const int before = last_sketch_stream.exchange(c.stream);
+    const bool pipelined = before >= 0 && before != c.stream;
+    if (c.keep_t)
+        c.cus = sketch_split_resolve(SketchSplitIn{n_cu, c.nb, c.d, c.n, c.s, c.lt, c.rt, left && c.aux != c.stream, pipelined,
+                                                   fused ? SKETCH_FUSED : SKETCH_OTHER}, set);
     if (!(c.st_aux = stream_of(c.aux))) return TTSK_ERR_ARG;
     if (!(c.ws0 = (double *)scratch(c.stream, SCRATCH_DRIVER, c.bytes))) return TTSK_ERR_HIP;
     int rc;
@@ -294,7 +324,7 @@
                 p.C[cidx] = nch == 1 ? psi : blk0 + (size_t)cidx * c.szPs;
             }
             const StreamSmallArgs ss{nch, 0 , (int)Kc, (int)r, p.A, ldt, p.B, ldr, p.C, r, nch == 1 ? c.accumulate : 0};
-            CK(psi_stream(stream_small_try, ss, l * nn, q, stream_of(q)));
+            CK(psi_stream(stream_small_try, ss, l * nn, q, stream_of(q), c.cus.psi));
             if (rc == 1) return nch > 1 ? ttsk_sum_slices(psi, blk0, nch, c.szPs, (size_t)(l * nn * r), c.accumulate, q) : TTSK_OK;
         }
     }
@@ -329,7 +359,7 @@
                 TTSK_HIP(hipMemset2DAsync(c.Tp0(0, mu) + t_len, c.szT[mu] * 8, 0, 8, (size_t)nb, stq));
             const StreamSmallSumArgs sa{nb, 0 , (int)sp, (int)r, c.Tslice(0, mu), ldt, (int64_t)c.szT[mu],
                                         c.Rslice(0, jr), ldr, (int64_t)c.szR[jr], c.out + c.psi_at[mu], r, c.accumulate};
-            CK(psi_stream(stream_small_sum_try, sa, l * nn, q, stq));
+            CK(psi_stream(stream_small_sum_try, sa, l * nn, q, stq, c.cus.psi));
         }
         if (rc == 0) {
             double *blk0 = c.Ps(mu & 1);
@@ -338,7 +368,7 @@
             }
             const int acc = c.sum ? 0 : c.accumulate;
             const StreamSmallArgs ss{nb, 0 , (int)sp, (int)r, p.A, ldt, p.B, ldr, p.C, r, acc};
-            CK(psi_stream(stream_small_try, ss, l * nn, q, stq));
+            CK(psi_stream(stream_small_try, ss, l * nn, q, stq, c.cus.psi));
             if (rc == 0) CK(gemm_batch(4, nb, gemm_desc2(l * nn, r, 1, sp, ldt, 0, 1, 0, ldr, 1, r, 1, acc), p, q, stq));
             if (c.sum) CK(ttsk_sum_slices(c.out + c.psi_at[mu], blk0, nb, c.szPs, (size_t)(l * nn * r), c.accumulate, q));
         }
@@ -375,7 +405,7 @@
             p.A[cnt] = c.Tslice(b, mu); p.B[cnt] = c.Rslice(b, d - 2 - mu); p.C[cnt] = c.outb(b) + c.psi_at[mu];
         }
     const StreamSmallArgs ss{cnt, 0 , (int)sp, (int)r, p.A, c.t_ld(1), p.B, ldr, p.C, r, c.accumulate};
-    CK(psi_stream(stream_small_try, ss, l * nn, c.stream, c.st));
+    CK(psi_stream(stream_small_try, ss, l * nn, c.stream, c.st, c.cus.psi));
     if (rc == 0) return 0;
     BatchPtrs o{};
     cnt = 0;
@@ -427,7 +457,7 @@
         }
     }
     const StreamSmallArgs ss{cnt, 0 , (int)Kc, (int)r, p.A, ldt, p.B, ldr, p.C, r, 0};
-    CK(psi_stream(stream_small_try, ss, l * nn, c.stream, c.st));
+    CK(psi_stream(stream_small_try, ss, l * nn, c.stream, c.st, c.cus.psi));
     if (rc == 0) return TTSK_OK;
     psi_batched = true;
     CK(ttsk_stream_wait(c.aux, c.stream));
@@ -447,6 +477,14 @@
                             const int64_t *r_lo, const int64_t *r_hi)
 {
     return sketch_offsets(d, n, l_lo, l_hi, r_lo, r_hi);
+}
+
+int ttsk_tt_sketch_split(int right_cus, int left_cus, int psi_cus)
+{
+    TTSK_ARG(right_cus >= -1 && left_cus >= -1 && psi_cus >= -1, "ttsk_tt_sketch_split: budgets (%d, %d, %d) must be >= -1", right_cus,
+             left_cus, psi_cus);
+    split_set[0] = right_cus; split_set[1] = left_cus; split_set[2] = psi_cus;
+    return TTSK_OK;
 }
 
 int ttsk_tt_sketch(int d, const int64_t *n, const int64_t *s, const int64_t *lt, const int64_t *l_lo,
```

New measurement: 60400 (median of 6 runs). 1.03x the previous value.
